# AcrylicShrimp/omok-ai

Hardware: AMD Instinct MI355X
Metric: self-play games/sec (15x15, 800 sims/move); MCTS nodes/sec (higher is better)
Workload: dtype f16x3 split MFMA, fp32 acc; fc0 corrections mixed f16/fp6; 1 GPU; 4096 concurrent 15x15 games per GPU, 800 sims/move, K=16, two trees per game; games_per_gpu=4096, board=15, sims_per_move=800, batch_k=16, warmup_step=whole episode, parallelism=games sharded x1, no hot-path collective

## Files before the change

### bindings/omok_mi355x.rs

```rust
#![allow(non_camel_case_types, dead_code)]

use std::ffi::{CStr, CString};
use std::os::raw::{c_char, c_int, c_void};
use std::ptr;

#[repr(C)]
#[derive(Clone, Copy, Debug)]
pub struct OmokConfig {
    pub board_size: i32,
    pub games: i32,
    pub max_nodes: i32,
    pub max_tables: i32,
    pub max_batch_k: i32,
    pub device: i32,
    pub net_mode: i32,
    pub max_tree_waves: i32,
    pub seed: u64,
    pub game_offset: i64,
}

#[repr(C)]
pub struct OmokEngine {
    _private: [u8; 0],
}
// ... 104 lines not shown
        pub fn omok_advance(e: *mut OmokEngine) -> c_int;
        pub fn omok_compute_policy(e: *mut OmokEngine, pi: *mut f32, has_policy: *mut u8) -> c_int;
        pub fn omok_play_actions(e: *mut OmokEngine, actions: *const i32) -> c_int;
        pub fn omok_set_actions(e: *mut OmokEngine, actions: *const i32) -> c_int;
        pub fn omok_selfplay_run(e: *mut OmokEngine, count: i32, batch_size: i32, epsilon: f32, alpha: f32, temperature: f32, threshold: i32, max_plies: i32, stats: *mut f64) -> c_int;
        pub fn omok_env_scripted_actions(e: *mut OmokEngine, kind: i32, boards: *const u8, turns: *const u8, batch: i32, forced_out: *mut i32) -> c_int;
        pub fn omok_opponent_actions(e: *mut OmokEngine, kind: i32, actions: *mut i32) -> c_int;
        pub fn omok_versus_run(e: *mut OmokEngine, kind: i32, opponent_side: i32, count: i32, batch_size: i32, epsilon: f32, alpha: f32, max_plies: i32, results: *mut i32, stats: *mut f64) -> c_int;
        pub fn omok_selfplay_run_slots(e: *mut OmokEngine, total_games: i32, count: i32, batch_size: i32, epsilon: f32, alpha: f32, temperature: f32, threshold: i32, records_dev: *mut c_void, cap_records: i64, game_offsets: *mut i64, game_lengths: *mut i32, game_status: *mut i32, n_records: *mut i64, stats: *mut f64) -> c_int;
        pub fn omok_round_generate(e: *mut OmokEngine, round: i32, batch_size: i32, epsilon: f32, alpha: f32, n_requests: *mut i32) -> c_int;
        pub fn omok_round_inputs(e: *mut OmokEngine, inputs: *mut f32) -> c_int;
        pub fn omok_round_eval(e: *mut OmokEngine) -> c_int;
        pub fn omok_round_outputs(e: *mut OmokEngine, p: *mut f32, v: *mut f32) -> c_int;
        pub fn omok_round_logits(e: *mut OmokEngine, logits: *mut f32, vpre: *mut f32) -> c_int;
        pub fn omok_round_inject(e: *mut OmokEngine, p: *const f32, v: *const f32) -> c_int;
        pub fn omok_round_scatter(e: *mut OmokEngine) -> c_int;
        pub fn omok_mirror_generate(e: *mut OmokEngine, n_requests: *mut i32) -> c_int;
        pub fn omok_mirror_inputs(e: *mut OmokEngine, inputs: *mut f32) -> c_int;
        pub fn omok_mirror_eval(e: *mut OmokEngine) -> c_int;
        pub fn omok_mirror_outputs(e: *mut OmokEngine, p: *mut f32) -> c_int;
        pub fn omok_mirror_inject(e: *mut OmokEngine, p: *const f32) -> c_int;
        pub fn omok_mirror_apply(e: *mut OmokEngine) -> c_int;
        pub fn omok_train_begin(e: *mut OmokEngine, max_batch: i32) -> c_int;
        pub fn omok_train_end(e: *mut OmokEngine) -> c_int;
        pub fn omok_train_step(e: *mut OmokEngine, records_dev: *const c_void, n_records: i64, indices: *const i64, batch: i32, losses: *mut f32) -> c_int;
        pub fn omok_train_losses(e: *mut OmokEngine, records_dev: *const c_void, n_records: i64, indices: *const i64, batch: i32, losses: *mut f32) -> c_int;
        pub fn omok_train_batch_indices(e: *mut OmokEngine, n_records: i64, batch: i32, key: u64, step: i32, out: *mut i64) -> c_int;
        pub fn omok_train_run(e: *mut OmokEngine, records_dev: *const c_void, n_records: i64, update_count: i32, batch_size: i32, key: u64, losses: *mut f32) -> c_int;
        pub fn omok_train_gradient_count(e: *const OmokEngine) -> i64;
        pub fn omok_train_backward(e: *mut OmokEngine, records_dev: *const c_void, n_records: i64, indices: *const i64, batch: i32, grad_dst_dev: *mut c_void) -> c_int;
        pub fn omok_train_apply(e: *mut OmokEngine, grads_dev: *const c_void, ranks: i32, losses: *mut f32) -> c_int;
        pub fn omok_debug_train_gradient(e: *mut OmokEngine, index: i32, out: *mut f32, count: i64) -> c_int;
        pub fn omok_net_read(e: *mut OmokEngine, index: i32, out: *mut f32, count: i64) -> c_int;
        pub fn omok_alive_count(e: *mut OmokEngine) -> c_int;
        pub fn omok_current_ply(e: *mut OmokEngine) -> c_int;
        pub fn omok_game_info(e: *mut OmokEngine, alive: *mut u8, status: *mut u8, plies: *mut i32) -> c_int;
        pub fn omok_tree_dump(e: *mut OmokEngine, game: i32, side: i32, ints: *mut i32, floats: *mut f32, cap_nodes: i32) -> c_int;
        pub fn omok_tree_root(e: *mut OmokEngine, game: i32, side: i32, root_n: *mut u32, root_w: *mut f32, n_nodes: *mut i32, n_tables: *mut i32) -> c_int;
        pub fn omok_root_stats(e: *mut OmokEngine, n: *mut u32, w: *mut f32) -> c_int;
        pub fn omok_root_children(e: *mut OmokEngine, game: i32, side: i32, actions: *mut i32, n: *mut u32, w: *mut f32, p: *mut f32, cap: i32) -> c_int;
        pub fn omok_replay_game(e: *mut OmokEngine, game: i32, boards: *mut u8, turns: *mut u8, pi: *mut f32, z: *mut f32, cap_plies: i32) -> c_int;
        pub fn omok_game_log_enable(e: *mut OmokEngine, enabled: i32) -> c_int;
        pub fn omok_game_log_read(e: *mut OmokEngine, first_game: i32, games: i32, start_boards: *mut u8, lengths: *mut i32, moves: *mut u16, root_n: *mut u32, root_w: *mut f32, child_n: *mut u32, child_w: *mut f32) -> c_int;
        pub fn omok_env_replay(e: *mut OmokEngine, start_boards: *const u8, moves: *const u16, lengths: *const i32, batch: i32, stride: i32, upto: i32, boards_out: *mut u8, status_out: *mut i32, played_out: *mut i32) -> c_int;
        pub fn omok_replay_pack_dev(e: *mut OmokEngine, dst_dev: *mut c_void, cap_records: i64) -> i64;
        pub fn omok_replay_record_bytes(e: *const OmokEngine) -> i32;
        pub fn omok_replay_augment_dev(e: *mut OmokEngine, dst_dev: *mut c_void, cap_records: i64) -> i64;
        pub fn omok_replay_augmented_game(e: *mut OmokEngine, game: i32, boards: *mut u8, turns: *mut u8, pi: *mut f32, z: *mut f32, cap_records: i32) -> c_int;
        pub fn omok_operand_row_bytes(e: *const OmokEngine) -> i64;
        pub fn omok_debug_operand_rows(e: *mut OmokEngine, first_row: i32, rows: i32, out: *mut c_void) -> c_int;
        pub fn omok_debug_set_base_cache(e: *mut OmokEngine, enabled: i32) -> c_int;
        pub fn omok_debug_set_children_kernel(e: *mut OmokEngine, which: i32) -> c_int;
        pub fn omok_debug_set_window_rects(e: *mut OmokEngine, enabled: i32) -> c_int;
        pub fn omok_debug_last_plan(e: *mut OmokEngine, out: *mut i32, cap: i32) -> c_int;
        pub fn omok_get_stats(e: *mut OmokEngine, stats: *mut f64) -> c_int;
        pub fn omok_reset_stats(e: *mut OmokEngine) -> c_int;
        pub fn omok_set_profiling(e: *mut OmokEngine, enabled: i32) -> c_int;
    }
}


#[repr(u8)]
#[derive(Clone, Copy, Debug, PartialEq, Eq)]
pub enum GameStatus {
    InProgress = 0,
    Draw = 1,
    BlackWin = 2,
    WhiteWin = 3,
}

impl GameStatus {
    pub fn from_raw(v: i32) -> Option<GameStatus> {
        match v {
            0 => Some(GameStatus::InProgress),
            1 => Some(GameStatus::Draw),
            2 => Some(GameStatus::BlackWin),
            3 => Some(GameStatus::WhiteWin),
            _ => None,
        }
    }
}

#[derive(Debug)]
pub struct OmokError {
    pub code: i32,
    pub message: String,
}

pub struct Engine {
    raw: *mut OmokEngine,
    hw: usize,
    games: usize,
}
unsafe impl Send for Engine {}

impl Engine {
    fn check(&self, rc: c_int) -> Result<c_int, OmokError> {
        if rc >= 0 {
            return Ok(rc);
        }
        let message = unsafe { CStr::from_ptr(ffi::omok_last_error(self.raw)) }.to_string_lossy().into_owned();
        Err(OmokError { code: rc, message })
    }

    pub fn new(cfg: &OmokConfig) -> Result<Engine, OmokError> {
        let mut raw: *mut OmokEngine = ptr::null_mut();
// ... 122 lines not shown
```

### include/omok_mi355x.h

```cpp
#ifndef OMOK_MI355X_H
#define OMOK_MI355X_H
#include <stdint.h>

#ifdef __cplusplus
extern "C" {
#endif

#define OMOK_OK 0
#define OMOK_ERR_INVALID (-1)
#define OMOK_ERR_HIP (-2)
#define OMOK_ERR_STATE (-3)
#define OMOK_ERR_OVERFLOW (-4)
#define OMOK_ERR_ILLEGAL (-5)

#define OMOK_MODE_PLAYER 0
#define OMOK_MODE_OPPONENT 1

#define OMOK_NET_F16X3 0
#define OMOK_NET_F32 1
#define OMOK_NET_F16X3_ROWS 2

#define OMOK_NET_F16X3_FP6 3
#define OMOK_NET_F16X3_F16 4
#define OMOK_NET_F16X3_MIXED 5
// ... 80 lines not shown
int omok_round_eval(omok_engine* e);
int omok_round_outputs(omok_engine* e, float* p, float* v);
int omok_round_logits(omok_engine* e, float* logits, float* vpre);
int omok_round_inject(omok_engine* e, const float* p, const float* v);
int omok_round_scatter(omok_engine* e);
int omok_mirror_generate(omok_engine* e, int32_t* n_requests);
int omok_mirror_inputs(omok_engine* e, float* inputs);
int omok_mirror_eval(omok_engine* e);
int omok_mirror_outputs(omok_engine* e, float* p);
int omok_mirror_inject(omok_engine* e, const float* p);
int omok_mirror_apply(omok_engine* e);

int omok_train_begin(omok_engine* e, int32_t max_batch);
int omok_train_end(omok_engine* e);
int omok_train_step(omok_engine* e, const void* records_dev, int64_t n_records, const int64_t* indices, int32_t batch, float* losses);
int omok_train_losses(omok_engine* e, const void* records_dev, int64_t n_records, const int64_t* indices, int32_t batch, float* losses);
int omok_train_batch_indices(omok_engine* e, int64_t n_records, int32_t batch, uint64_t key, int32_t step, int64_t* out);
int omok_train_run(omok_engine* e, const void* records_dev, int64_t n_records, int32_t update_count, int32_t batch_size, uint64_t key, float* losses);
#define OMOK_TRAIN_MAX_RANKS 64
int64_t omok_train_gradient_count(const omok_engine* e);
int omok_train_backward(omok_engine* e, const void* records_dev, int64_t n_records, const int64_t* indices, int32_t batch, void* grad_dst_dev);
int omok_train_apply(omok_engine* e, const void* grads_dev, int32_t ranks, float* losses);
int omok_debug_train_gradient(omok_engine* e, int32_t index, float* out, int64_t count);
int omok_net_read(omok_engine* e, int32_t index, float* out, int64_t count);

int omok_alive_count(omok_engine* e);
int omok_current_ply(omok_engine* e);
int omok_game_info(omok_engine* e, uint8_t* alive, uint8_t* status, int32_t* plies);
int omok_tree_dump(omok_engine* e, int32_t game, int32_t side, int32_t* ints, float* floats, int32_t cap_nodes);
int omok_tree_root(omok_engine* e, int32_t game, int32_t side, uint32_t* root_n, float* root_w,
                   int32_t* n_nodes, int32_t* n_tables);
int omok_root_stats(omok_engine* e, uint32_t* n, float* w);
int omok_root_children(omok_engine* e, int32_t game, int32_t side, int32_t* actions, uint32_t* n, float* w, float* p, int32_t cap);
int omok_replay_game(omok_engine* e, int32_t game, uint8_t* boards, uint8_t* turns, float* pi, float* z,
                     int32_t cap_plies);
#define OMOK_MOVE_CELL 255
#define OMOK_MOVE_EXTERNAL 256
int omok_game_log_enable(omok_engine* e, int32_t enabled);
int omok_game_log_read(omok_engine* e, int32_t first_game, int32_t games, uint8_t* start_boards, int32_t* lengths, uint16_t* moves,
                       uint32_t* root_n, float* root_w, uint32_t* child_n, float* child_w);
int omok_env_replay(omok_engine* e, const uint8_t* start_boards, const uint16_t* moves, const int32_t* lengths, int32_t batch,
                    int32_t stride, int32_t upto, uint8_t* boards_out, int32_t* status_out, int32_t* played_out);
int64_t omok_replay_pack_dev(omok_engine* e, void* dst_dev, int64_t cap_records);
int32_t omok_replay_record_bytes(const omok_engine* e);
int64_t omok_replay_augment_dev(omok_engine* e, void* dst_dev, int64_t cap_records);
int omok_replay_augmented_game(omok_engine* e, int32_t game, uint8_t* boards, uint8_t* turns, float* pi, float* z,
                               int32_t cap_records);

int64_t omok_operand_row_bytes(const omok_engine* e);
int omok_debug_operand_rows(omok_engine* e, int32_t first_row, int32_t rows, void* out);
int omok_debug_set_base_cache(omok_engine* e, int32_t enabled);
int omok_debug_set_children_kernel(omok_engine* e, int32_t which);
int omok_debug_set_window_rects(omok_engine* e, int32_t enabled);
#define OMOK_PLAN_INTS 16
int omok_debug_last_plan(omok_engine* e, int32_t* out, int32_t cap);

#define OMOK_STAT_SIMS 0
#define OMOK_STAT_EVALS 1
#define OMOK_STAT_PLY_GAMES 2
#define OMOK_STAT_FINISHED 3
#define OMOK_STAT_MS_TREE 4
#define OMOK_STAT_MS_TRUNK 5
#define OMOK_STAT_MS_FC0 6
#define OMOK_STAT_MS_TAIL 7
#define OMOK_STAT_MS_PLY 8
#define OMOK_STAT_FC0_LAUNCHES 9
#define OMOK_STAT_FC0_ROWS 10
#define OMOK_STAT_TREE_BYTES 11
#define OMOK_STAT_ROUND_LAUNCHES 12
#define OMOK_STAT_MS_ROUND 13
#define OMOK_STAT_PEAK_NODES 14
#define OMOK_STAT_PEAK_TABLES 15
#define OMOK_STAT_FC0_FORMAT 16
#define OMOK_STAT_PROBE_ROWS 17
#define OMOK_STAT_PROBE_DP_FP6 18
#define OMOK_STAT_PROBE_DV_FP6 19
#define OMOK_STAT_PROBE_DP_F16 20
#define OMOK_STAT_PROBE_DV_F16 21
#define OMOK_STAT_PROBE_LIMIT 22
#define OMOK_STAT_PROBE_LOGIT_MAX 23
#define OMOK_STAT_CHILDREN2_LAUNCHES 24
#define OMOK_STAT_CHILDREN1_LAUNCHES 25
#define OMOK_STAT_PROBE_DLOGIT_FP6 26
#define OMOK_STAT_PROBE_DLOGIT_F16 27
#define OMOK_STAT_PROBE_ROUND_ROWS 28
#define OMOK_STAT_PROBE_ROUND_FP6 29
#define OMOK_STAT_PROBE_ROUND_MIXED 32
#define OMOK_STAT_PROBE_ROUND_F16 35
#define OMOK_STAT_PROBE_LOGIT_LIMIT 38
#define OMOK_STAT_PROBE_OUTSIDE 39
#define OMOK_STAT_WORK_DIFF_RUNS 40
#define OMOK_STAT_WORK_DIFF_SINGLES 41
#define OMOK_STAT_WORK_DIFF_CHILDREN 42
#define OMOK_STAT_WORK_COPY_RUNS 43
#define OMOK_STAT_WORK_COPY_SINGLES 44
#define OMOK_STAT_WORK_COPY_CHILDREN 45
#define OMOK_STAT_WORK_DIFF_FULL_RUNS 46
#define OMOK_STAT_WORK_WIN_PIXELS 47
#define OMOK_STAT_WORK_WIN_TILES 48
#define OMOK_STAT_WORK_FULL_TILES 49
#define OMOK_STAT_MS_TRAIN_APPLY 50
#define OMOK_STAT_COUNT 51
int omok_get_stats(omok_engine* e, double* stats );
int omok_reset_stats(omok_engine* e);
int omok_set_profiling(omok_engine* e, int32_t enabled);

// ... 5 lines not shown
```

### omok-ai_amd/api.py

```python
import ctypes as C

import os

import numpy as np

from . import binding as B
from . import weights as W

EMPTY, BLACK, WHITE = 0, 1, 2
TURN_BLACK, TURN_WHITE = 0, 1
IN_PROGRESS, DRAW, BLACK_WIN, WHITE_WIN = 0, 1, 2, 3


class Engine:

    def __init__(self, board_size=15, games=1, max_nodes=2048, max_tables=1024, max_batch_k=16, device=0,
                 net_mode=B.NET_F16X3, seed=0, game_offset=0, max_tree_waves=0):
        self.n, self.hw, self.games = board_size, board_size * board_size, games
        self.max_nodes = max_nodes
        self.max_batch_k = max_batch_k
        cfg = B.Config(board_size, games, max_nodes, max_tables, max_batch_k, device, net_mode, max_tree_waves, seed, game_offset)
        h = C.c_void_p()
        rc = B.lib().omok_create(C.byref(cfg), C.byref(h))
        if rc != 0:
# ... 157 lines not shown
        forced = np.zeros(len(boards), dtype=np.int32)
        self._chk(B.lib().omok_env_scripted_actions(self.h, int(kind), B.u8ptr(boards), B.u8ptr(turns), len(boards), B.iptr(forced)))
        return forced

    def env_check_positions(self, boards):
        boards = np.ascontiguousarray(boards, dtype=np.uint8).reshape(-1, self.hw)
        verdict = np.zeros(len(boards), dtype=np.int32)
        stones = np.zeros(len(boards), dtype=np.int32)
        self._chk(B.lib().omok_env_check_positions(self.h, B.u8ptr(boards), len(boards), B.iptr(verdict), B.iptr(stones)))
        return verdict, stones

    def env_random_positions(self, key, first_game, stones, batch):
        boards = np.zeros((int(batch), self.hw), dtype=np.uint8)
        ok = np.zeros(int(batch), dtype=np.uint8)
        self._chk(B.lib().omok_env_random_positions(self.h, int(key) & 0xFFFFFFFFFFFFFFFF, int(first_game), int(stones), int(batch),
                                                    B.u8ptr(boards), B.u8ptr(ok)))
        return boards, ok

    def env_replay(self, start_boards, moves, lengths, upto=-1):
        moves = np.ascontiguousarray(moves, dtype=np.uint16)
        lengths = np.ascontiguousarray(lengths, dtype=np.int32).reshape(-1)
        batch = len(lengths)
        moves = moves.reshape(batch, -1)
        start = None
        if start_boards is not None:
            start = np.ascontiguousarray(start_boards, dtype=np.uint8).reshape(batch, self.hw)
        boards = np.zeros((batch, self.hw), dtype=np.uint8)
        status = np.zeros(batch, dtype=np.int32)
        played = np.zeros(batch, dtype=np.int32)
        self._chk(B.lib().omok_env_replay(self.h, None if start is None else B.u8ptr(start), moves.ctypes.data_as(C.POINTER(C.c_uint16)),
                                          B.iptr(lengths), batch, moves.shape[1], int(upto), B.u8ptr(boards), B.iptr(status), B.iptr(played)))
        return boards, status, played

    def encode_nn_input(self, boards, turns, mode=B.MODE_PLAYER):
        boards = np.ascontiguousarray(boards, dtype=np.uint8).reshape(-1, self.hw)
        turns = np.ascontiguousarray(turns, dtype=np.uint8).reshape(-1)
        out = np.zeros((boards.shape[0], 3 * self.hw), dtype=np.float32)
        self._chk(B.lib().omok_encode_nn_input(self.h, B.u8ptr(boards), B.u8ptr(turns), boards.shape[0], mode, B.fptr(out)))
        return out.reshape(-1, self.n, self.n, 3)

    def operand_rows(self, first_row, rows):
        nb = int(B.lib().omok_operand_row_bytes(self.h))
        if nb < 0:
            raise B.OmokError(nb, "no operand rows in this net mode")
        out = np.empty((rows, nb), dtype=np.uint8)
        self._chk(B.lib().omok_debug_operand_rows(self.h, first_row, rows, out.ctypes.data_as(C.c_void_p)))
        return out

    def set_base_cache(self, on=True):
        self._chk(B.lib().omok_debug_set_base_cache(self.h, int(bool(on))))

    def set_window_rects(self, on=True):
        self._chk(B.lib().omok_debug_set_window_rects(self.h, int(bool(on))))

    def set_children_kernel(self, which=2):
        self._chk(B.lib().omok_debug_set_children_kernel(self.h, int(which)))

    def last_plan(self):
        out = np.zeros(len(B.PLAN_NAMES), dtype=np.int32)
        n = self._chk(B.lib().omok_debug_last_plan(self.h, B.iptr(out), out.size))
        assert n == out.size
        d = dict(zip(B.PLAN_NAMES, (int(x) for x in out)))
        d["path"] = B.PLAN_PATHS[d["path"]]
        return d

    def set_profiling(self, on=True):
        self._chk(B.lib().omok_set_profiling(self.h, int(on)))

    def stats(self):
        s = (C.c_double * len(B.STAT_NAMES))()
        self._chk(B.lib().omok_get_stats(self.h, s))
        return dict(zip(B.STAT_NAMES, list(s)))

    def reset_stats(self):
        self._chk(B.lib().omok_reset_stats(self.h))


class Environment:

    def __init__(self, engine):
        self.eng = engine
        self._board = np.zeros((1, engine.hw), dtype=np.uint8)
        self._turn = np.zeros(1, dtype=np.uint8)
        self._legal = np.full(1, engine.hw, dtype=np.uint16)

    board = property(lambda s: s._board[0])
    turn = property(lambda s: int(s._turn[0]))
    legal_move_count = property(lambda s: int(s._legal[0]))

    def place_stone(self, index):
        s = int(self.eng.env_place_stone(self._board, self._turn, self._legal, [int(index)])[0])
        return None if s < 0 else s

    @staticmethod
    def check_positions(engine, boards):
        return engine.env_check_positions(boards)

    @staticmethod
    def random_positions(engine, key, first_game, stones, batch):
        return engine.env_random_positions(key, first_game, stones, batch)

    def encode_board(self, turn):
        t = np.array([turn], dtype=np.uint8)
        return self.eng.encode_nn_input(self.board[None], t, B.MODE_PLAYER).reshape(-1)[: 2 * self.eng.hw].copy()


# ... 271 lines not shown
```

### omok-ai_amd/binding.py

```python
import ctypes as C
import os
import subprocess

import numpy as np

_HERE = os.path.dirname(os.path.abspath(__file__))
LIB_PATH = os.environ.get("OMOK_MI355X_LIB") or os.path.join(_HERE, "libomok_mi355x.so")

OK = 0
NET_F16X3, NET_F32, NET_F16X3_ROWS, NET_F16X3_FP6, NET_F16X3_F16, NET_F16X3_MIXED = 0, 1, 2, 3, 4, 5
FC0_FORMATS = {-1: "f32", 0: "fp6", 1: "f16", 2: "mixed"}
MODE_PLAYER, MODE_OPPONENT = 0, 1
OPP_RANDOM, OPP_NAIVE = 0, 1
PLAN_NAMES = ["path", "rows", "nsplit", "tsplit", "runs", "singles", "run_rows", "full_runs", "tiles", "t_split", "ways", "fways",
              "fc0_format", "n_cu", "nsup", "reserved"]
PLAN_PATHS = {-1: "none", 0: "plain", 1: "copy", 2: "difference", 3: "f32"}
STAT_NAMES = ["sims", "evals", "ply_games", "finished", "ms_tree", "ms_trunk", "ms_fc0", "ms_tail", "ms_ply",
              "fc0_launches", "fc0_rows", "tree_bytes", "round_launches", "ms_round", "peak_nodes", "peak_tables",
              "fc0_format", "probe_rows", "probe_dp_fp6", "probe_dv_fp6", "probe_dp_f16", "probe_dv_f16", "probe_limit", "probe_logit_max",
              "children2_launches", "children1_launches", "probe_dlogit_fp6", "probe_dlogit_f16", "probe_round_rows",
              "probe_round_dp_fp6", "probe_round_dv_fp6", "probe_round_dlogit_fp6", "probe_round_dp_mixed", "probe_round_dv_mixed", "probe_round_dlogit_mixed",
              "probe_round_dp_f16", "probe_round_dv_f16", "probe_round_dlogit_f16", "probe_logit_limit", "probe_outside",
              "work_diff_runs", "work_diff_singles", "work_diff_children", "work_copy_runs", "work_copy_singles", "work_copy_children", "work_diff_full_runs",
              "work_win_pixels", "work_win_tiles", "work_full_tiles", "ms_train_apply"]

SYMBOLS = [
    "omok_create", "omok_destroy", "omok_last_error", "omok_net_num_tensors", "omok_net_tensor_size", "omok_net_load",
    "omok_net_commit", "omok_net_load_file", "omok_net_save_file", "omok_net2_load", "omok_net2_commit", "omok_net2_load_file", "omok_net2_info", "omok_match_reset", "omok_evaluate_pv", "omok_evaluate_logits", "omok_env_play", "omok_env_place_stone", "omok_encode_nn_input", "omok_selfplay_reset", "omok_set_episode", "omok_execute", "omok_execute_shared", "omok_execute_shared_recorded",
    "omok_compute_policy", "omok_play_actions", "omok_set_actions", "omok_root_children",
    "omok_env_scripted_actions", "omok_opponent_actions", "omok_versus_run",
    "omok_env_check_positions", "omok_selfplay_reset_from", "omok_root_stats",
    "omok_match_reset_from", "omok_env_random_positions",
    "omok_sample_actions", "omok_advance", "omok_selfplay_run", "omok_selfplay_run_slots", "omok_round_generate", "omok_round_inputs",
    "omok_round_eval", "omok_round_outputs", "omok_round_logits", "omok_round_inject", "omok_round_scatter", "omok_mirror_generate",
    "omok_mirror_inputs", "omok_mirror_eval", "omok_mirror_outputs", "omok_mirror_inject", "omok_mirror_apply",
    "omok_alive_count", "omok_current_ply", "omok_game_info", "omok_tree_dump", "omok_tree_root", "omok_replay_game",
    "omok_operand_row_bytes", "omok_debug_operand_rows", "omok_debug_set_base_cache", "omok_debug_set_children_kernel", "omok_debug_set_window_rects", "omok_debug_last_plan",
    "omok_replay_pack_dev", "omok_replay_record_bytes", "omok_replay_augment_dev", "omok_replay_augmented_game", "omok_get_stats", "omok_reset_stats", "omok_set_profiling",
    "omok_train_begin", "omok_train_end", "omok_train_step", "omok_train_losses", "omok_train_batch_indices", "omok_train_run",
    "omok_train_gradient_count", "omok_train_backward", "omok_train_apply",
    "omok_debug_train_gradient", "omok_net_read",
    "omok_game_log_enable", "omok_game_log_read", "omok_env_replay",
]


class Config(C.Structure):
    _fields_ = [("board_size", C.c_int32), ("games", C.c_int32), ("max_nodes", C.c_int32), ("max_tables", C.c_int32),
                ("max_batch_k", C.c_int32), ("device", C.c_int32), ("net_mode", C.c_int32), ("max_tree_waves", C.c_int32),
                ("seed", C.c_uint64), ("game_offset", C.c_int64)]


class OmokError(RuntimeError):
    def __init__(self, code, msg):
        super().__init__(f"omok error {code}: {msg}")
        self.code = code


def build():
    subprocess.check_call(["make", "-s", "-C", os.path.join(_HERE, "csrc")])


_lib = None


def lib():
    global _lib
    if _lib is not None:
        return _lib
    if not os.path.exists(LIB_PATH):
        raise OmokError(-2, f"{LIB_PATH} is missing: build it with __graft_entry__.build() (hipcc --offload-arch=gfx950); "
                            "there is no CPU fallback")
    L = C.CDLL(LIB_PATH)
    fp, ip = C.POINTER(C.c_float), C.POINTER(C.c_int32)
    u8p = C.POINTER(C.c_uint8)
    H = C.c_void_p
    L.omok_create.argtypes = [C.POINTER(Config), C.POINTER(H)]
    L.omok_destroy.argtypes = [H]
    L.omok_destroy.restype = None
    L.omok_last_error.argtypes = [H]
    L.omok_last_error.restype = C.c_char_p
    L.omok_net_tensor_size.argtypes = [H, C.c_int]
    L.omok_net_tensor_size.restype = C.c_int64
    L.omok_net_load.argtypes = [H, C.c_int, fp, C.c_int64]
    L.omok_net_commit.argtypes = [H]
    L.omok_net_load_file.argtypes = [H, C.c_char_p]
    L.omok_net_save_file.argtypes = [H, C.c_char_p]
    L.omok_net2_load.argtypes = [H, C.c_int, fp, C.c_int64]
    L.omok_net2_commit.argtypes = [H]
    L.omok_net2_load_file.argtypes = [H, C.c_char_p]
    L.omok_net2_info.argtypes = [H, ip, ip, C.POINTER(C.c_double)]
    L.omok_match_reset.argtypes = [H, C.c_int32]
    L.omok_evaluate_pv.argtypes = [H, fp, C.c_int32, fp, fp]
    L.omok_evaluate_logits.argtypes = [H, fp, C.c_int32, fp, fp]
    L.omok_env_play.argtypes = [H, ip, C.c_int32, C.c_int32, ip, u8p, u8p, C.POINTER(C.c_uint16)]
    L.omok_encode_nn_input.argtypes = [H, u8p, u8p, C.c_int32, C.c_int32, fp]
    L.omok_selfplay_reset.argtypes = [H]
    L.omok_execute_shared_recorded.argtypes = [H, C.c_int32, C.c_int32, C.c_float, C.c_float, C.c_int32, u8p, u8p, ip, fp, fp, C.c_int32, ip, ip]
    L.omok_operand_row_bytes.argtypes = [H]
    L.omok_operand_row_bytes.restype = C.c_int64
    L.omok_debug_operand_rows.argtypes = [H, C.c_int32, C.c_int32, C.c_void_p]
    L.omok_debug_set_base_cache.argtypes = [H, C.c_int32]
    L.omok_debug_set_children_kernel.argtypes = [H, C.c_int32]
    L.omok_debug_set_window_rects.argtypes = [H, C.c_int32]
    L.omok_debug_last_plan.argtypes = [H, ip, C.c_int32]
    L.omok_set_episode.argtypes = [H, C.c_uint64]
    L.omok_env_place_stone.argtypes = [H, u8p, u8p, C.POINTER(C.c_uint16), ip, C.c_int32, ip]
    L.omok_compute_policy.argtypes = [H, fp, u8p]
    L.omok_play_actions.argtypes = [H, ip]
    L.omok_set_actions.argtypes = [H, ip]
    L.omok_env_scripted_actions.argtypes = [H, C.c_int32, u8p, u8p, C.c_int32, ip]
    L.omok_opponent_actions.argtypes = [H, C.c_int32, ip]
    L.omok_versus_run.argtypes = [H, C.c_int32, C.c_int32, C.c_int32, C.c_int32, C.c_float, C.c_float, C.c_int32, ip, C.POINTER(C.c_double)]
    L.omok_env_check_positions.argtypes = [H, u8p, C.c_int32, ip, ip]
    L.omok_selfplay_reset_from.argtypes = [H, u8p]
    L.omok_match_reset_from.argtypes = [H, C.c_int32, u8p]
    L.omok_env_random_positions.argtypes = [H, C.c_uint64, C.c_int64, C.c_int32, C.c_int32, u8p, u8p]
    L.omok_root_stats.argtypes = [H, C.POINTER(C.c_uint32), fp]
    L.omok_root_children.argtypes = [H, C.c_int32, C.c_int32, ip, C.POINTER(C.c_uint32), fp, fp, C.c_int32]
    L.omok_execute.argtypes = [H, C.c_int32, C.c_int32, C.c_float, C.c_float]
    L.omok_execute_shared.argtypes = [H, C.c_int32, C.c_int32, C.c_float, C.c_float, C.c_int32]
    L.omok_sample_actions.argtypes = [H, C.c_float, C.c_int32, ip]
    L.omok_advance.argtypes = [H]
    L.omok_selfplay_run.argtypes = [H, C.c_int32, C.c_int32, C.c_float, C.c_float, C.c_float, C.c_int32, C.c_int32,
                                    C.POINTER(C.c_double)]
    L.omok_selfplay_run_slots.argtypes = [H, C.c_int32, C.c_int32, C.c_int32, C.c_float, C.c_float, C.c_float, C.c_int32, C.c_void_p, C.c_int64,
                                          C.POINTER(C.c_int64), ip, ip, C.POINTER(C.c_int64), C.POINTER(C.c_double)]
    L.omok_round_generate.argtypes = [H, C.c_int32, C.c_int32, C.c_float, C.c_float, ip]
    L.omok_round_inputs.argtypes = [H, fp]
    L.omok_round_eval.argtypes = [H]
    L.omok_round_outputs.argtypes = [H, fp, fp]
    L.omok_round_logits.argtypes = [H, fp, fp]
    L.omok_round_inject.argtypes = [H, fp, fp]
    L.omok_round_scatter.argtypes = [H]
    L.omok_mirror_generate.argtypes = [H, ip]
    L.omok_mirror_inputs.argtypes = [H, fp]
    L.omok_mirror_eval.argtypes = [H]
    L.omok_mirror_outputs.argtypes = [H, fp]
    L.omok_mirror_inject.argtypes = [H, fp]
    L.omok_mirror_apply.argtypes = [H]
    L.omok_alive_count.argtypes = [H]
    L.omok_current_ply.argtypes = [H]
    L.omok_game_info.argtypes = [H, u8p, u8p, ip]
    L.omok_tree_dump.argtypes = [H, C.c_int32, C.c_int32, ip, fp, C.c_int32]
    L.omok_tree_root.argtypes = [H, C.c_int32, C.c_int32, C.POINTER(C.c_uint32), fp, ip, ip]
    L.omok_replay_game.argtypes = [H, C.c_int32, u8p, u8p, fp, fp, C.c_int32]
    L.omok_replay_pack_dev.argtypes = [H, C.c_void_p, C.c_int64]
    L.omok_replay_pack_dev.restype = C.c_int64
    L.omok_replay_augment_dev.argtypes = [H, C.c_void_p, C.c_int64]
    L.omok_replay_augment_dev.restype = C.c_int64
    L.omok_replay_augmented_game.argtypes = [H, C.c_int32, u8p, u8p, fp, fp, C.c_int32]
    L.omok_replay_record_bytes.argtypes = [H]
    L.omok_get_stats.argtypes = [H, C.POINTER(C.c_double)]
    L.omok_reset_stats.argtypes = [H]
    L.omok_set_profiling.argtypes = [H, C.c_int32]
    i64p = C.POINTER(C.c_int64)
    L.omok_train_begin.argtypes = [H, C.c_int32]
# ... 30 lines not shown
```

### omok-ai_amd/csrc/common.h

```cpp
#pragma once
#include <hip/hip_runtime.h>
#include <stdint.h>

namespace omok {

constexpr uint16_t NONE16 = 0xFFFFu;
constexpr uint8_t NONE8 = 0xFFu;
constexpr int KMAX = 64;
constexpr float F32_EPS = 1.1920928955078125e-7f;

enum { ST_IN_PROGRESS = 0, ST_DRAW = 1, ST_BLACK_WIN = 2, ST_WHITE_WIN = 3 };
enum { RNG_EXPAND = 1, RNG_NOISE = 2, RNG_SAMPLE = 3, RNG_OPPONENT = 4, RNG_TRAIN_BATCH = 5 };

template <int N>
struct Geo {
    static constexpr int HW = N * N;
    static constexpr int ROWP = (HW + 63) / 64 * 64;
    static constexpr int NW = (HW + 63) / 64;
    static constexpr int IT = ROWP / 64;
};

struct __attribute__((aligned(16))) NodeHdr {
    uint16_t parent;
    uint16_t table;
// ... 48 lines not shown
    uint32_t* req_aux;
    int32_t* d_count;
    uint64_t* rp_board;
    uint8_t* rp_turn;
    float* rp_pi;
    float* rp_z;
    unsigned long long* d_bytes;
    int cap_nodes, cap_tables, games;
    int stride_nodes, stride_tables;
};

struct RoundArgs {
    int side, round, K, ply;
    float epsilon, alpha;
    uint64_t seed;
    int64_t game_offset;
    const float* scatter_v;
};

void launch_reset(int n, const Store& S, const float* root_policy_dev , hipStream_t st);
void launch_reset_from(int n, const Store& S, const uint8_t* boards_dev, const float* p_dev, const float* p2_dev, int split, hipStream_t st);
void launch_random_positions(int n, uint64_t key, int64_t first_game, int stones, int batch, uint8_t* boards_dev, uint8_t* ok_dev, hipStream_t st);
void launch_position_check(int n, const uint8_t* boards_dev, int batch, int32_t* verdict_dev, int32_t* stones_dev, hipStream_t st);
struct GameLog {
    uint32_t* root_n;
    float* root_w;
    uint32_t* child_n;
    float* child_w;
    uint16_t* move;
    uint8_t* start_board;
};
void launch_log_move(int n, const Store& S, int side, int start_ply, const GameLog& L, hipStream_t st);
void launch_replay(int n, const uint8_t* start_dev, const int32_t* verdict_dev, const uint16_t* moves_dev, const int32_t* lengths_dev, int batch, int stride,
                   int upto, uint8_t* boards_out, int32_t* status_out, int32_t* played_out, hipStream_t st);
void launch_root_stats(const Store& S, int side, uint32_t* n_dev, float* w_dev, hipStream_t st);
struct SlotMeta { long long offset; int32_t len; int32_t status; };
void launch_harvest(int n, const Store& S, uint8_t* mask_dev , long long* slot_off_dev , long long* out_count_dev, SlotMeta* meta_dev,
                    uint8_t* dst_dev, long long cap_records, hipStream_t st);
void launch_refill(int n, const Store& S, const float* root_policy_dev, int32_t* next_gid_dev, int total_games, int32_t* new_gid_dev , hipStream_t st);
void launch_round(int n, const Store& S, const RoundArgs& a, hipStream_t st);
void launch_fill(const Store& S, int side, int K, hipStream_t st);
void launch_scan(int n, const Store& S, int side, int K, hipStream_t st, unsigned long long* evals_dev = nullptr, int32_t* zero_ptr = nullptr, int zero_n = 0,
                 bool fill = true);
void launch_round_shared(int n, const Store& S, const RoundArgs& a, int rounds_total, int group, int waves, uint16_t* sh_req, uint32_t* sh_cnt,
                         hipStream_t st, uint8_t* rec_order = nullptr, uint32_t* rec_pos = nullptr);
void launch_scatter_shared(int n, const Store& S, int side, const float* p_dev, const float* v_dev, int max_count, int waves, const uint16_t* sh_req,
                           const uint32_t* sh_cnt, hipStream_t st, uint8_t* rec_order = nullptr, uint32_t* rec_pos = nullptr);
constexpr int MAX_TREE_WAVES = 16;
constexpr int MAX_GAMES = 32767;
constexpr int SCAN_GAMES_PER_THREAD = 32;
void launch_scatter(int n, const Store& S, int side, const float* p_dev, const float* v_dev, int max_count, hipStream_t st, bool backups = true);
void launch_backups(int n, const Store& S, int side, const float* v_dev, hipStream_t st);
void launch_softmax_scatter(int n, const Store& S, int side, const float* logits_dev, int lrow, float* v_dev, float* vpre_dev, int max_count,
                            hipStream_t st, bool backups = true);
void launch_sample(int n, const Store& S, int side, int ply, float temperature, int threshold, uint64_t seed,
                   int64_t game_offset, int32_t* actions_dev, hipStream_t st);
void launch_mirror_scan(int n, const Store& S, int side, hipStream_t st);
void launch_advance(int n, const Store& S, int side, const float* p_dev, hipStream_t st);
void launch_encode_requests(int n, const Store& S, float* out_dev , int max_b, hipStream_t st);
void launch_env_play(int n, const int32_t* moves_dev, int batch, int len, int32_t* status_dev, uint8_t* boards_dev,
                     uint8_t* turns_dev, uint16_t* legal_dev, hipStream_t st);
void launch_encode_boards(int n, const uint8_t* boards_dev, const uint8_t* turns_dev, int batch, int mode,
                          float* out_dev, hipStream_t st);
void launch_replay_pack(int n, const Store& S, const long long* offsets_dev, uint8_t* dst_dev, long long cap_records, hipStream_t st);
void launch_replay_offsets(int n, const Store& S, int per_transition, long long* offsets_dev , hipStream_t st);
void launch_set_actions(int n, const Store& S, int side, const int32_t* actions_dev, uint32_t* d_flags , hipStream_t st);
void launch_clear_actions(const Store& S, hipStream_t st);
void launch_opponent_move(int n, const Store& S, int side, int kind, uint64_t seed, int64_t game_offset, int32_t* actions_dev, hipStream_t st);
void launch_env_scripted(int n, const uint8_t* boards_dev, int kind, int batch, int32_t* forced_dev, hipStream_t st);
void launch_policy(int n, const Store& S, int side, float* pi_dev , uint8_t* has_dev , hipStream_t st);
void launch_env_place(int n, uint8_t* boards_dev, uint8_t* turns_dev, uint16_t* legal_dev, const int32_t* actions_dev, int batch,
                      int32_t* status_dev, hipStream_t st);
int set_advance_lds_attribute(int n, size_t bytes);
void launch_replay_augment(int n, const Store& S, const long long* offsets_dev, int game_first, int game_count, long long base_sub,
                           uint8_t* dst_dev, long long cap_records, hipStream_t st);
size_t advance_lds_bytes(int cap_nodes, int cap_tables);

void launch_match_split(const Store& S, int tree_side, int split, uint32_t* ref2, uint32_t* aux2, int32_t* cnt, unsigned long long* evals, int max_rows,
                        hipStream_t st);
void launch_match_join(const int32_t* cnt, const float* v2, float* v1, const float* p2, float* p1, int rowp, int max_rows, hipStream_t st);
void launch_match_roots(int n, const Store& S, const float* root_policy2, int split, hipStream_t st);

struct NetBuffers;
}
```

### omok-ai_amd/csrc/engine.cpp

```cpp
#include "../../include/omok_mi355x.h"
#include "common.h"
#include "net.h"
#include "train.h"

#include <algorithm>
#include <cstdarg>
#include <cstdio>
#include <cstring>
#include <string>
#include <vector>

using namespace omok;

hipEvent_t Prof::get() {
    if (n_pool > 0) return pool[--n_pool];
    hipEvent_t e;
    hipEventCreate(&e);
    return e;
}
void Prof::begin(int cat, hipStream_t st) {
    if (!enabled || !active) return;
    if (n_items == cap_items) {
        if (cap_items >= 8192) resolve();
        else {
// ... 263 lines not shown
    rc |= dalloc(e, &e->d_sh_cnt, 2 * (size_t)KMAX);
    rc |= dalloc(e, &e->d_flags, 4);
    rc |= dalloc(e, &e->d_pi, G * HW);
    rc |= dalloc(e, &e->d_has, G);
    rc |= dalloc(e, &e->d_aug_offsets, G + 1);
    if (rc) {
        g_create_error = e->err;
        omok_destroy(e);
        return OMOK_ERR_HIP;
    }
    hipMemsetAsync(S.d_count, 0, 16, e->st);
    hipMemsetAsync(S.d_bytes, 0, 16, e->st);
    hipMemsetAsync(e->d_error, 0, 16, e->st);
    hipMemsetAsync(e->d_evals, 0, 16, e->st);
    hipMemsetAsync(S.gs, 0, sizeof(GameState) * G, e->st);
    hipMemsetAsync(S.ts, 0, sizeof(TreeState) * T, e->st);
    if (set_advance_lds_attribute(e->n, advance_lds_bytes(cfg->max_nodes, cfg->max_tables)) != 0) {
        g_create_error = "hipFuncSetAttribute(k_advance, max dynamic LDS) failed";
        omok_destroy(e);
        return OMOK_ERR_HIP;
    }
    configure_net(e, e->net, (int)max_b);
    if (net_alloc(e->net) == 0) {
        g_create_error = "net buffer allocation failed (hipMalloc)";
        omok_destroy(e);
        return OMOK_ERR_HIP;
    }
    if (hipStreamSynchronize(e->st) != hipSuccess) {
        g_create_error = "stream sync failed after init";
        omok_destroy(e);
        return OMOK_ERR_HIP;
    }
    *out = e;
    return OMOK_OK;
}

extern "C" int omok_net_num_tensors(void) { return NET_TENSORS; }
extern "C" int64_t omok_net_tensor_size(const omok_engine* e, int index) { return e ? net_tensor_size(e->n, index) : -1; }

static int sync_and_check(omok_engine* e, const char* what);

static int net2_alloc(omok_engine* e) {
    if (e->net2) return 0;
    const size_t mb = (size_t)e->net.max_b;
    if (!e->d_mref && dalloc(e, &e->d_mref, mb)) return OMOK_ERR_HIP;
    if (!e->d_maux && dalloc(e, &e->d_maux, mb)) return OMOK_ERR_HIP;
    if (!e->d_mcnt && dalloc(e, &e->d_mcnt, 4)) return OMOK_ERR_HIP;
    if (!e->d_mevals && dalloc(e, &e->d_mevals, 2)) return OMOK_ERR_HIP;
    if (!e->d_root_policy2 && dalloc(e, &e->d_root_policy2, (size_t)e->rowp)) return OMOK_ERR_HIP;
    HIPCHK(e, hipMemset(e->d_mcnt, 0, 16));
    HIPCHK(e, hipMemset(e->d_mevals, 0, 16));
    Net* n2 = new Net();
    configure_net(e, *n2, e->net.max_b);
    if (net_alloc(*n2) == 0) { delete n2; return fail(e, OMOK_ERR_HIP, "net 2 buffer allocation failed (hipMalloc)"); }
    e->net2 = n2;
    return 0;
}

static int net_load_slot(omok_engine* e, int slot, int index, const float* data, int64_t count) {
    if (!e || !data) return OMOK_ERR_INVALID;
    if (index < 0 || index >= NET_TENSORS) return fail(e, OMOK_ERR_INVALID, "tensor index %d out of range", index);
    if (count != e->net.wsize[index]) return fail(e, OMOK_ERR_INVALID, "tensor %d: expected %lld values, got %lld", index, (long long)e->net.wsize[index], (long long)count);
    HIPCHK(e, hipSetDevice(e->cfg.device));
    if (slot == 2 && net2_alloc(e)) return OMOK_ERR_HIP;
    Net& net = slot == 2 ? *e->net2 : e->net;
    HIPCHK(e, hipMemcpyAsync(net.w[index], data, sizeof(float) * (size_t)count, hipMemcpyHostToDevice, e->st));
    HIPCHK(e, hipStreamSynchronize(e->st));
    net.loaded[index] = true;
    net.committed = false;
    return OMOK_OK;
}

static int net_commit_slot(omok_engine* e, int slot) {
    if (!e) return OMOK_ERR_INVALID;
    if (slot == 2 && !e->net2) return fail(e, OMOK_ERR_STATE, "net 2: no tensor was ever loaded");
    Net& net = slot == 2 ? *e->net2 : e->net;
    for (int i = 0; i < NET_TENSORS; ++i)
        if (!net.loaded[i]) return fail(e, OMOK_ERR_STATE, "tensor %d was never loaded", i);
    HIPCHK(e, hipSetDevice(e->cfg.device));
    if (e->round_reqs >= 0 || e->mirror_reqs >= 0) return fail(e, OMOK_ERR_STATE, "omok_net_commit while a round / mirror batch is pending");
    if (net_commit(net, e->S, e->st) != 0) return fail(e, OMOK_ERR_HIP, "weight packing / format probe failed");
    net_invalidate_sibling_cache(net);
    HIPCHK(e, hipStreamSynchronize(e->st));
    net.committed = true;
    return OMOK_OK;
}

extern "C" int omok_net_load(omok_engine* e, int index, const float* data, int64_t count) { return net_load_slot(e, 1, index, data, count); }
extern "C" int omok_net_commit(omok_engine* e) { return net_commit_slot(e, 1); }
extern "C" int omok_net2_load(omok_engine* e, int index, const float* data, int64_t count) { return net_load_slot(e, 2, index, data, count); }
extern "C" int omok_net2_commit(omok_engine* e) { return net_commit_slot(e, 2); }

extern "C" int omok_net2_info(omok_engine* e, int32_t* fc0_format, int32_t* probe_outside, double* evals) {
    if (!e) return OMOK_ERR_INVALID;
    if (!e->net2 || !e->net2->committed) return fail(e, OMOK_ERR_STATE, "net 2 not loaded/committed (omok_net2_load x31 + omok_net2_commit)");
    ENTER(e);
    const Net& n2 = *e->net2;
    if (fc0_format) *fc0_format = n2.mode == OMOK_NET_F32 ? -1 : (n2.diff_fp6 ? FC0_MIXED : n2.fc0_fmt);
    if (probe_outside) *probe_outside = n2.probe_outside;
    if (evals) {
        unsigned long long ev[2] = {0, 0};
        if (sync_and_check(e, "net2_info")) return OMOK_ERR_HIP;
        HIPCHK(e, hipMemcpy(ev, e->d_mevals, sizeof(ev), hipMemcpyDeviceToHost));
        evals[0] = (double)ev[0];
        evals[1] = (double)ev[1];
    }
// ... 54 lines not shown
    }
    fclose(f);
    for (int i = 0; rc == OMOK_OK && i < NET_TENSORS; ++i) rc = net_load_slot(e, slot, i, params[i].data(), (int64_t)params[i].size());
    if (rc != OMOK_OK) return rc;
    return net_commit_slot(e, slot);
}
extern "C" int omok_net_load_file(omok_engine* e, const char* path) { return net_load_file_slot(e, 1, path); }
extern "C" int omok_net2_load_file(omok_engine* e, const char* path) { return net_load_file_slot(e, 2, path); }

extern "C" int omok_net_save_file(omok_engine* e, const char* path) {
    if (!e || !path) return OMOK_ERR_INVALID;
    for (int i = 0; i < NET_TENSORS; ++i)
        if (!e->net.loaded[i]) return fail(e, OMOK_ERR_STATE, "tensor %d was never loaded", i);
    HIPCHK(e, hipSetDevice(e->cfg.device));
    FILE* f = fopen(path, "wb");
    if (!f) return fail(e, OMOK_ERR_INVALID, "cannot create weights file %s", path);
    bool ok = wr_u64(f, NET_TENSORS);
    char name[64];
    for (int i = 0; ok && i < NET_TENSORS; ++i) {
        net_tensor_name(i, name, sizeof(name));
        const size_t len = strlen(name);
        ok = wr_u64(f, len) && fwrite(name, 1, len, f) == len;
    }
    ok = ok && wr_u64(f, NET_TENSORS);
    std::vector<float> buf;
    for (int i = 0; ok && i < NET_TENSORS; ++i) {
        const size_t len = (size_t)e->net.wsize[i];
        buf.resize(len);
        if (hipMemcpy(buf.data(), e->net.w[i], sizeof(float) * len, hipMemcpyDeviceToHost) != hipSuccess) { fclose(f); return fail(e, OMOK_ERR_HIP, "weight read-back failed"); }
        ok = wr_u64(f, len) && fwrite(buf.data(), sizeof(float), len, f) == len;
    }
    ok = (fclose(f) == 0) && ok;
    return ok ? OMOK_OK : fail(e, OMOK_ERR_INVALID, "short write to %s", path);
}

static int need_net(omok_engine* e) {
    if (!e->net.committed) return fail(e, OMOK_ERR_STATE, "net not loaded/committed (omok_net_load x31 + omok_net_commit)");
    if (e->match && !e->net2->committed) return fail(e, OMOK_ERR_STATE, "match episode: net 2 was reloaded and not committed (omok_net2_commit)");
    return 0;
}

static Net& net_at(omok_engine* e, int idx) { return idx == 0 ? e->net : *e->net2; }
static void invalidate_nets(omok_engine* e) {
    net_invalidate_sibling_cache(e->net);
    if (e->net2) net_invalidate_sibling_cache(*e->net2);
}
static bool block_live(const omok_engine* e, int b) { return b == 0 ? e->split > 0 : e->split < e->cfg.games; }
static Store block_view(const omok_engine* e, int b) {
    Store V = e->S;
    if (b == 0) V.d_count = e->d_mcnt;
    else { V.req_ref = e->d_mref; V.req_aux = e->d_maux; V.d_count = e->d_mcnt + 1; }
    return V;
}
static void match_forward(omok_engine* e, int b, int tree_side, int max_count, int sibling_side, bool skip_softmax) {
    Net& X = net_at(e, tree_side ^ b);
    X.grp_lo = b ? e->split : 0;
    X.grp_hi = b ? e->cfg.games : e->split;
    X.grp_sub = b ? e->d_mcnt : nullptr;
    net_forward_requests(X, block_view(e, b), max_count, e->st, &e->prof, sibling_side, skip_softmax);
    X.grp_hi = -1;
    X.grp_sub = nullptr;
}
static void match_split(omok_engine* e, int tree_side, int max_rows) {
    launch_match_split(e->S, tree_side, e->split, e->d_mref, e->d_maux, e->d_mcnt, e->d_mevals, max_rows, e->st);
}
static void match_join(omok_engine* e, int tree_side, bool p, int max_rows) {
    if (!block_live(e, 1)) return;
    Net &A = net_at(e, tree_side), &B = net_at(e, tree_side ^ 1);
    launch_match_join(e->d_mcnt, B.v, A.v, p ? B.p : nullptr, p ? A.p : nullptr, e->rowp, max_rows, e->st);
}
static int match_counts(omok_engine* e) {
    HIPCHK(e, hipMemcpyAsync(e->match_cnt, e->d_mcnt, sizeof(e->match_cnt), hipMemcpyDeviceToHost, e->st));
    return sync_and_check(e, "match counts") ? OMOK_ERR_HIP : 0;
}
static int no_match(omok_engine* e, const char* what) {
    if (e->match) return fail(e, OMOK_ERR_STATE, "%s is not available in a match episode (omok_match_reset): start self-play with omok_selfplay_reset", what);
    return 0;
}

static int check_async(omok_engine* e, const char* what) {
    hipError_t r = hipGetLastError();
    if (r != hipSuccess) return fail(e, OMOK_ERR_HIP, "%s: launch failed: %s", what, hipGetErrorString(r));
    return 0;
}

static int sync_and_check(omok_engine* e, const char* what) {
    hipError_t r = hipStreamSynchronize(e->st);
    if (r != hipSuccess) return fail(e, OMOK_ERR_HIP, "%s: %s", what, hipGetErrorString(r));
    return check_async(e, what);
}

extern "C" int omok_net_read(omok_engine* e, int32_t index, float* out, int64_t count) {
    if (!e || !out) return OMOK_ERR_INVALID;
    if (index < 0 || index >= NET_TENSORS) return fail(e, OMOK_ERR_INVALID, "tensor index %d out of range", index);
    if (count != e->net.wsize[index]) return fail(e, OMOK_ERR_INVALID, "tensor %d: expected %lld values, got %lld", index, (long long)e->net.wsize[index], (long long)count);
    if (!e->net.loaded[index]) return fail(e, OMOK_ERR_STATE, "tensor %d was never loaded", index);
    ENTER(e);
    if (sync_and_check(e, "net_read")) return OMOK_ERR_HIP;
    HIPCHK(e, hipMemcpy(out, e->net.w[index], sizeof(float) * (size_t)count, hipMemcpyDeviceToHost));
    return OMOK_OK;
}

extern "C" int omok_train_end(omok_engine* e) {
    ENTER(e);
    if (!e->train) return OMOK_OK;
    if (sync_and_check(e, "train_end")) return OMOK_ERR_HIP;
    train_free(*e->train);
    delete e->train;
    e->train = nullptr;
    return OMOK_OK;
}

extern "C" int omok_train_begin(omok_engine* e, int32_t max_batch) {
    if (!e) return OMOK_ERR_INVALID;
// ... 387 lines not shown
}

extern "C" int omok_selfplay_reset_from(omok_engine* e, const uint8_t* boards) {
    if (!e || !boards) return OMOK_ERR_INVALID;
    if (!e->net.committed) return fail(e, OMOK_ERR_STATE, "net not loaded/committed (omok_net_load x31 + omok_net_commit)");
    ENTER(e);
    return reset_from_positions(e, boards, false, 0);
}

extern "C" int omok_match_reset_from(omok_engine* e, int32_t split, const uint8_t* boards) {
    if (!e || !boards) return OMOK_ERR_INVALID;
    if (!e->net.committed) return fail(e, OMOK_ERR_STATE, "net not loaded/committed (omok_net_load x31 + omok_net_commit)");
    if (!e->net2 || !e->net2->committed) return fail(e, OMOK_ERR_STATE, "net 2 not loaded/committed (omok_net2_load x31 + omok_net2_commit)");
    if (split < 0 || split > e->cfg.games) return fail(e, OMOK_ERR_INVALID, "split %d outside [0, games = %d]", split, e->cfg.games);
    ENTER(e);
    return reset_from_positions(e, boards, true, split);
}

extern "C" int omok_env_random_positions(omok_engine* e, uint64_t key, int64_t first_game, int32_t stones, int32_t batch, uint8_t* boards_out,
                                         uint8_t* ok_out) {
    if (!e || !boards_out || !ok_out) return OMOK_ERR_INVALID;
    if (stones < 0 || stones >= e->hw) return fail(e, OMOK_ERR_INVALID, "stones %d outside [0, %d)", stones, e->hw);
    if (batch < 1) return fail(e, OMOK_ERR_INVALID, "batch %d < 1", batch);
    ENTER(e);
    uint8_t* d_out = nullptr;
    const size_t B = (size_t)batch;
    HIPCHK(e, hipMalloc((void**)&d_out, B * e->hw + B));
    e->prof.begin(PC_PLY, e->st);
    launch_random_positions(e->n, key, first_game, stones, batch, d_out, d_out + B * e->hw, e->st);
    e->prof.end(e->st);
    hipMemcpyAsync(boards_out, d_out, B * e->hw, hipMemcpyDeviceToHost, e->st);
    hipMemcpyAsync(ok_out, d_out + B * e->hw, B, hipMemcpyDeviceToHost, e->st);
    const int rc = sync_and_check(e, "env_random_positions");
    hipFree(d_out);
    return rc ? OMOK_ERR_HIP : OMOK_OK;
}

static int need_reset(omok_engine* e) {
    if (!e->reset_done) return fail(e, OMOK_ERR_STATE, "omok_selfplay_reset has not been called");
    return 0;
}

static void enqueue_match_round(omok_engine* e, int side, int K, bool eval_and_scatter, int alive, bool defer_backups) {
    const int max_req = std::min(alive * K, e->net.max_b);
    launch_scan(e->n, e->S, side, K, e->st, e->d_evals);
    match_split(e, side, max_req);
    e->prof.end(e->st);
    if (!eval_and_scatter) return;
    for (int b = 0; b < 2; ++b) {
        if (!block_live(e, b)) continue;
        Net& X = net_at(e, side ^ b);
        const Store V = block_view(e, b);
        const bool fused = net_logits_cover_batch(X, alive * K);
        match_forward(e, b, side, alive * K, side, fused);
        e->prof.begin(PC_TREE_OTHER, e->st);
        if (fused) {
            int lrow = 0;
            const float* lg = net_logits(X, &lrow);
            launch_softmax_scatter(e->n, V, side, lg, lrow, X.v, X.vpre, alive * K, e->st, false);
        } else launch_scatter(e->n, V, side, X.p, X.v, alive * K, e->st, false);
        e->prof.end(e->st);
    }
    e->prof.begin(PC_TREE_OTHER, e->st);
    match_join(e, side, false, max_req);
    if (!defer_backups) launch_backups(e->n, e->S, side, net_at(e, side).v, e->st);
    e->prof.end(e->st);
}

static Net& backup_net(omok_engine* e, int side) { return e->match ? net_at(e, side) : e->net; }

static void enqueue_round(omok_engine* e, int round, int K, float eps, float alpha, bool eval_and_scatter, int alive, bool defer_backups = false,
                          bool pending_backups = false) {
    const int side = e->ply & 1;
    RoundArgs a{side, round, K, e->ply, eps, alpha, e->key, e->cfg.game_offset, pending_backups ? backup_net(e, side).v : nullptr};
    e->prof.round_begin();
    e->prof.begin(PC_ROUND, e->st);
    launch_round(e->n, e->S, a, e->st);
    e->prof.end(e->st);
    e->prof.begin(PC_TREE_OTHER, e->st);
    if (e->match) {
        enqueue_match_round(e, side, K, eval_and_scatter, alive, defer_backups);
        e->prof.round_end();
        return;
    }
    int max_req = alive * K;
    if (max_req > e->net.max_b) max_req = e->net.max_b;
    const bool sib_round = eval_and_scatter && net_round_takes_sibling_path(e->net, max_req);
    launch_scan(e->n, e->S, side, K, e->st, e->d_evals, sib_round ? e->net.d_gcnt : nullptr, NET_GCNT_INTS, !sib_round);
    e->net.gcnt_zeroed = e->net.fill_in_group = sib_round;
    e->net.fill_side = side;
    e->net.fill_k = K;
    e->prof.end(e->st);
    if (eval_and_scatter) {
        const bool fused = net_logits_cover_batch(e->net, alive * K);
        net_forward_requests(e->net, e->S, alive * K, e->st, &e->prof, side, fused);
        e->prof.begin(PC_TREE_OTHER, e->st);
        if (fused) {
            int lrow = 0;
            const float* lg = net_logits(e->net, &lrow);
            launch_softmax_scatter(e->n, e->S, side, lg, lrow, e->net.v, e->net.vpre, alive * K, e->st, !defer_backups);
        } else launch_scatter(e->n, e->S, side, e->net.p, e->net.v, alive * K, e->st, !defer_backups);
        e->prof.end(e->st);
    }
    e->prof.round_end();
}

static int enqueue_execute(omok_engine* e, int count, int K, float eps, float alpha, int alive) {
    int processed = 0, round = 0;
    while (processed < count) {
        enqueue_round(e, round, K, eps, alpha, true, alive, true, round > 0);
        processed += K;
        round += 1;
    }
    if (round > 0) {
        e->prof.begin(PC_TREE_OTHER, e->st);
        launch_backups(e->n, e->S, e->ply & 1, backup_net(e, e->ply & 1).v, e->st);
        e->prof.end(e->st);
    }
    return round;
}

static int check_exec_args(omok_engine* e, int count, int K, float eps, float alpha) {
    if (count < 1) return fail(e, OMOK_ERR_INVALID, "count must be >= 1");
    if (K < 1 || K > e->cfg.max_batch_k) return fail(e, OMOK_ERR_INVALID, "batch_size %d outside [1, max_batch_k=%d]", K, e->cfg.max_batch_k);
    if (!(alpha > 0.0f)) return fail(e, OMOK_ERR_INVALID, "alpha must be > 0");
    if (!(eps >= 0.0f && eps <= 1.0f)) return fail(e, OMOK_ERR_INVALID, "epsilon must be in [0,1]");
    return 0;
}

extern "C" int omok_execute(omok_engine* e, int32_t count, int32_t batch_size, float epsilon, float alpha) {
    if (!e) return OMOK_ERR_INVALID;
    if (need_net(e) || need_reset(e)) return OMOK_ERR_STATE;
    if (check_exec_args(e, count, batch_size, epsilon, alpha)) return OMOK_ERR_INVALID;
    HIPCHK(e, hipSetDevice(e->cfg.device));
    uint32_t bits = 0, alive = 0;
    if (read_status(e, &bits, &alive)) return OMOK_ERR_HIP;
    const int rounds = enqueue_execute(e, count, batch_size, epsilon, alpha, (int)alive);
    e->sims += (double)rounds * batch_size * alive;
    if (read_status(e, &bits, &alive)) return OMOK_ERR_HIP;
    return tree_error(e, bits);
}

extern "C" int omok_execute_shared(omok_engine* e, int32_t count, int32_t batch_size, float epsilon, float alpha, int32_t waves) {
    if (!e) return OMOK_ERR_INVALID;
    if (need_net(e) || need_reset(e)) return OMOK_ERR_STATE;
    if (check_exec_args(e, count, batch_size, epsilon, alpha)) return OMOK_ERR_INVALID;
    if (no_match(e, "omok_execute_shared")) return OMOK_ERR_STATE;
    if (e->cfg.games != 1) return fail(e, OMOK_ERR_INVALID, "omok_execute_shared searches ONE tree: create the engine with games = 1 (got %d)", e->cfg.games);
    if (waves < 1 || waves > MAX_TREE_WAVES || waves * batch_size > e->net.max_b)
        return fail(e, OMOK_ERR_INVALID, "waves must be in [1, %d] and waves * batch_size <= %d (the net batch, sized by max(games, max_tree_waves = %d) * max_batch_k)",
                    MAX_TREE_WAVES, e->net.max_b, e->cfg.max_tree_waves);
    HIPCHK(e, hipSetDevice(e->cfg.device));
    uint32_t bits = 0, alive = 0;
// ... 908 lines not shown
    launch_replay_offsets(e->n, e->S, 6, e->d_aug_offsets, e->st);
    launch_replay_augment(e->n, e->S, e->d_aug_offsets, 0, e->cfg.games, 0, (uint8_t*)dst_dev, cap_records, e->st);
    long long total = 0;
    if (hipMemcpyAsync(&total, e->d_aug_offsets + e->cfg.games, 8, hipMemcpyDeviceToHost, e->st) != hipSuccess) return OMOK_ERR_HIP;
    if (sync_and_check(e, "replay_augment")) return OMOK_ERR_HIP;
    return total;
}

extern "C" int omok_replay_augmented_game(omok_engine* e, int32_t game, uint8_t* boards, uint8_t* turns, float* pi, float* z, int32_t cap_records) {
    if (!e || game < 0 || game >= e->cfg.games || cap_records < 0) return OMOK_ERR_INVALID;
    HIPCHK(e, hipSetDevice(e->cfg.device));
    const size_t hw = (size_t)e->hw, brd = (hw + 1 + 3) / 4 * 4, rec = brd + 4 * hw + 4, max_rec = 6 * hw;
    if (!e->d_aug_scratch && dalloc(e, &e->d_aug_scratch, max_rec * rec)) return OMOK_ERR_HIP;
    long long off[2] = {0, 0};
    launch_replay_offsets(e->n, e->S, 6, e->d_aug_offsets, e->st);
    HIPCHK(e, hipMemcpyAsync(off, e->d_aug_offsets + game, 16, hipMemcpyDeviceToHost, e->st));
    if (sync_and_check(e, "replay_augmented_game")) return OMOK_ERR_HIP;
    const int total = (int)(off[1] - off[0]);
    const int n = total < cap_records ? total : cap_records;
    if (n <= 0) return total;
    launch_replay_augment(e->n, e->S, e->d_aug_offsets, game, 1, off[0], e->d_aug_scratch, (long long)max_rec, e->st);
    std::vector<uint8_t> host((size_t)total * rec);
    HIPCHK(e, hipMemcpyAsync(host.data(), e->d_aug_scratch, host.size(), hipMemcpyDeviceToHost, e->st));
    if (sync_and_check(e, "replay_augmented_game")) return OMOK_ERR_HIP;
    for (int i = 0; i < n; ++i) {
        const uint8_t* r = host.data() + (size_t)i * rec;
        if (boards) memcpy(boards + (size_t)i * hw, r, hw);
        if (turns) turns[i] = r[hw];
        if (pi) memcpy(pi + (size_t)i * hw, r + brd, 4 * hw);
        if (z) memcpy(z + i, r + brd + 4 * hw, 4);
    }
    return total;
}

extern "C" int64_t omok_operand_row_bytes(const omok_engine* e) { return e && e->net.mode != OMOK_NET_F32 ? (int64_t)e->net.row_u4 * 16 : OMOK_ERR_INVALID; }
extern "C" int omok_debug_operand_rows(omok_engine* e, int32_t first_row, int32_t rows, void* out) {
    if (!e || !out || first_row < 0 || rows < 0 || first_row + rows > e->net.max_b || e->net.mode == OMOK_NET_F32) return OMOK_ERR_INVALID;
    ENTER(e);
    HIPCHK(e, hipMemcpyAsync(out, (const char*)e->net.a_fc0 + (size_t)first_row * e->net.row_u4 * 16, (size_t)rows * e->net.row_u4 * 16, hipMemcpyDeviceToHost, e->st));
    return sync_and_check(e, "debug_operand_rows") ? OMOK_ERR_HIP : OMOK_OK;
}

extern "C" int omok_debug_set_base_cache(omok_engine* e, int32_t enabled) {
    if (!e) return OMOK_ERR_INVALID;
    e->net.base_cache = enabled != 0;
    net_invalidate_sibling_cache(e->net);
    return OMOK_OK;
}

extern "C" int omok_debug_set_window_rects(omok_engine* e, int32_t enabled) {
    if (!e) return OMOK_ERR_INVALID;
    e->net.win_rects = enabled != 0;
    return OMOK_OK;
}

extern "C" int omok_debug_set_children_kernel(omok_engine* e, int32_t which) {
    if (!e) return OMOK_ERR_INVALID;
    if (which != 1 && which != 2) return fail(e, OMOK_ERR_INVALID, "children kernel %d (1 = k_sib_children, 2 = k_sib_children2)", which);
    if (which == 1 && e->net.mode != OMOK_NET_F32 && e->net.diff_fp6)
        return fail(e, OMOK_ERR_STATE, "omok_debug_set_children_kernel(1): the engine runs the mixed operand format, whose difference path exists in k_sib_children2 only "
                                       "(create the engine with OMOK_NET_F16X3_FP6 or _F16 to compare the two kernels)");
    e->net.sib_v2 = which == 2;
    net_invalidate_sibling_cache(e->net);
    return OMOK_OK;
}

extern "C" int omok_debug_last_plan(omok_engine* e, int32_t* out, int32_t cap) {
    if (!e || !out || cap < 0) return OMOK_ERR_INVALID;
    ENTER(e);
    const Net& net = e->net;
    int32_t plan[OMOK_PLAN_INTS] = {};
    plan[0] = net.plan_path; plan[1] = net.plan_rows; plan[2] = net.plan_nsplit; plan[3] = net.plan_tsplit;
    plan[12] = net.mode == OMOK_NET_F32 ? -1 : net.diff_fp6 ? FC0_MIXED : net.fc0_fmt;
    plan[13] = net.n_cu;
    plan[14] = 2 * net.hw;
    if (sync_and_check(e, "debug_last_plan")) return OMOK_ERR_HIP;
    if ((net.plan_path == 1 || net.plan_path == 2) && net.d_gcnt) {
        int32_t c[NET_GCNT_HEAD_INTS];
        HIPCHK(e, hipMemcpy(c, net.d_gcnt, sizeof(c), hipMemcpyDeviceToHost));
        plan[4] = c[NET_GCNT_RUNS]; plan[5] = c[NET_GCNT_SINGLES]; plan[6] = c[NET_GCNT_ROWS_IN_RUNS];
        if (net.plan_path == 2) {
            plan[7] = c[NET_GCNT_FULL_EVALS]; plan[8] = c[NET_GCNT_WIN_TILES]; plan[9] = c[NET_GCNT_SPLIT_TILE0]; plan[10] = c[NET_GCNT_WIN_WAYS];
            plan[11] = c[NET_GCNT_FULL_WAYS];
        }
    }
    const int n = cap < OMOK_PLAN_INTS ? cap : OMOK_PLAN_INTS;
    for (int i = 0; i < n; ++i) out[i] = plan[i];
    return n;
}

extern "C" int omok_get_stats(omok_engine* e, double* stats) {
    if (!e || !stats) return OMOK_ERR_INVALID;
    HIPCHK(e, hipSetDevice(e->cfg.device));
    if (sync_and_check(e, "get_stats")) return OMOK_ERR_HIP;
    e->prof.resolve();
    unsigned long long ev = 0, by = 0;
    HIPCHK(e, hipMemcpy(&ev, e->d_evals, 8, hipMemcpyDeviceToHost));
    HIPCHK(e, hipMemcpy(&by, e->S.d_bytes, 8, hipMemcpyDeviceToHost));
    for (int i = 0; i < OMOK_STAT_COUNT; ++i) stats[i] = 0.0;
    stats[OMOK_STAT_SIMS] = e->sims;
    stats[OMOK_STAT_EVALS] = e->evals + (double)ev;
    stats[OMOK_STAT_PLY_GAMES] = e->ply_games;
    stats[OMOK_STAT_FINISHED] = e->finished;
    stats[OMOK_STAT_MS_TREE] = e->prof.total_ms(PC_ROUND) + e->prof.total_ms(PC_TREE_OTHER);
    stats[OMOK_STAT_MS_TRUNK] = e->prof.total_ms(PC_TRUNK);
    stats[OMOK_STAT_MS_FC0] = e->prof.total_ms(PC_FC0);
// ... 59 lines not shown
```

### omok-ai_amd/csrc/net.h

```cpp
#pragma once
#include "common.h"
#include "../../include/omok_mi355x.h"

namespace omok {

constexpr int NET_TENSORS = 31;
constexpr int NC = 128;
constexpr int NM = 32;
constexpr int NF = 512;
enum { FC0_AUTO = -1, FC0_FP6 = 0, FC0_F16 = 1, FC0_MIXED = 2 };
constexpr float NET_PROBE_LIMIT = 3e-4f;
constexpr float NET_PROBE_LOGIT_LIMIT = 5e-4f;
constexpr float NET_PROBE_CONTRACT = 1e-3f;
constexpr int NET_PROBE_ROWS = 2048;

struct Net {
    int n = 0, hw = 0, rowp = 0, mode = 0;
    int cfg_mode = 0;
    bool siblings = true;
    int device = 0;
    int max_b = 0;
    bool committed = false;
    bool loaded[NET_TENSORS] = {};
    int64_t wsize[NET_TENSORS] = {};
    float* w[NET_TENSORS] = {};
    float* p = nullptr;
    float* v = nullptr;
    float* vpre = nullptr;
    float* in_f32 = nullptr;
    int chunk = 0;
    float *sx = nullptr, *sh = nullptr, *sd = nullptr, *sg = nullptr, *s0 = nullptr, *s1 = nullptr;
    float *s0_x3 = nullptr, *s0_f32 = nullptr;
    int probe_outside = 0;
    void* wt_trunk = nullptr;
    float* wt_first = nullptr;
    void* wt_fc0 = nullptr;
    void* wt_fc1 = nullptr;
    void* wt_heads = nullptr;
    void* a_fc0 = nullptr;
    void* h0 = nullptr;
    size_t row_u4 = 0;
    size_t part_rows = 0;
    float* part = nullptr;
    void* d_groups = nullptr;
    int32_t* d_singles = nullptr;
    void* d_sib_rows = nullptr;
    int32_t* d_gcnt = nullptr;
    unsigned long long* d_work = nullptr;
    float* sib_h = nullptr;
    uint32_t* d_sib_slot = nullptr;
    int32_t* d_bin_start = nullptr;
    int32_t* d_tile_info = nullptr;
    void* d_slot_desc = nullptr;
    void* d_rows = nullptr;
    size_t d_slots = 0;
    int games = 0;
    size_t base_slots = 0;
    void* a_base = nullptr;
    float* facc = nullptr;
    int32_t* d_tags = nullptr;
    void* d_comp = nullptr;
    bool gcnt_zeroed = false;
    bool fill_in_group = false;
    int fill_side = 0, fill_k = 0;
    double children_launches[2] = {0.0, 0.0};
    bool sib_v2 = true;
    bool win_rects = true;
    bool base_cache = true;
    bool sib_cache_valid = false;
    float* part_w = nullptr;
    size_t part_w_rows = 0;
    int n_cu = 256;
    int mx_sw = 0;
    int fc0_policy = FC0_AUTO;
    int fc0_fmt = 0;
    bool diff_fp6 = false;
    void* wt_fc0x = nullptr;
    size_t row_u4_fmt[2] = {0, 0};
    float probe[24] = {};
    size_t bytes = 0;
    int grp_lo = 0, grp_hi = -1;
    const int32_t* grp_sub = nullptr;
    int plan_path = -1, plan_rows = 0, plan_nsplit = 0, plan_tsplit = 0;
};

inline int64_t net_tensor_size(int n, int idx) {
    const int64_t hw = (int64_t)n * n;
    if (idx == 0) return 3 * NC;
    if (idx == 1) return NC;
    if (idx >= 2 && idx < 23) {
        const int64_t q[7] = {NC * NM, NM, 9 * NM, NM * NM, NM, NM * NC, NC};
        return q[(idx - 2) % 7];
    }
    switch (idx) {
        case 23: return NC * hw * NF;
        case 24: return NF;
        case 25: return (int64_t)NF * NF;
        case 26: return NF;
        case 27: return NF;
        case 28: return 1;
        case 29: return NF * hw;
        case 30: return hw;
    }
    return -1;
}

bool net_logits_cover_batch(const Net& net, int max_count);
bool net_round_takes_sibling_path(const Net& net, int max_count);
enum {
    NET_GCNT_RUNS = 0,
    NET_GCNT_SINGLES = 1,
    NET_GCNT_ROWS_IN_RUNS = 2,
    NET_GCNT_FULL_ROWS = 3,
    NET_GCNT_WIN_TILES = 4,
    NET_GCNT_SPLIT_TILE0 = 5,
    NET_GCNT_WIN_WAYS = 6,
    NET_GCNT_TILE_ORDER = 7,
    NET_GCNT_BINS = 8,
    NET_GCNT_FULL_EVALS = 96,
    NET_GCNT_UNCACHEABLE = 97,
    NET_GCNT_FULL_WAYS = 98,
    NET_GCNT_FULL_STRIDE = 99,
    NET_GCNT_HEAD_INTS = 100
};
constexpr int NET_GCNT_P0 = 8 + 81 + 7 + 16;
constexpr int NET_GCNT_INTS = NET_GCNT_P0 + 225;
constexpr int NET_WORK_DIFF = 0, NET_WORK_COPY = 3, NET_WORK_DIFF_FULL = 6, NET_WORK_WIN_PIXELS = 7, NET_WORK_WIN_TILES = 8, NET_WORK_FULL_TILES = 9, NET_WORK_COUNT = 16;
void net_forward_requests(Net& net, const Store& S, int max_count, hipStream_t st, struct Prof* prof, int sibling_side = -1, bool skip_softmax = false);
void net_forward_inputs(Net& net, const Store& S, int count, hipStream_t st, struct Prof* prof);
inline void net_invalidate_sibling_cache(Net& net) { net.sib_cache_valid = false; }
int net_commit(Net& net, const Store& S, hipStream_t st);
void net_set_fc0_format(Net& net, int fmt);
const float* net_logits(const Net& net, int* row_stride);
size_t net_alloc(Net& net);
void net_free(Net& net);

enum { PC_ROUND = 0, PC_TREE_OTHER, PC_TRUNK, PC_FC0, PC_TAIL, PC_PLY, PC_TRAIN_APPLY, PC_COUNT };
constexpr int PC_COUNT_MAX = 8;
struct Prof {
    bool enabled = false;
    int every = 1;
    long long rounds_seen = 0, rounds_timed = 0;
    bool active = true;
    bool in_round = false;
    double ms_s[PC_COUNT_MAX] = {};
    long long launches_s[PC_COUNT_MAX] = {};
    void round_begin() { in_round = true; active = every <= 1 || rounds_seen % every == 0; ++rounds_seen; if (active) ++rounds_timed; }
    void round_end() { in_round = false; active = true; }
    double scale() const { return rounds_timed > 0 ? (double)rounds_seen / (double)rounds_timed : 1.0; }
    double total_ms(int cat) const { return ms[cat] + ms_s[cat] * scale(); }
    double total_launches(int cat) const { return (double)launches[cat] + (double)launches_s[cat] * scale(); }
    struct Item { int cat; bool sampled; hipEvent_t a, b; };
    Item* items = nullptr;
    int n_items = 0, cap_items = 0;
    hipEvent_t* pool = nullptr;
    int n_pool = 0, cap_pool = 0;
    double ms[PC_COUNT] = {};
    long long launches[PC_COUNT] = {};
    hipEvent_t get();
    void begin(int cat, hipStream_t st);
    void end(hipStream_t st);
    void resolve();
    void destroy();
};

}
```

### omok-ai_amd/csrc/net_kernels.hip

```cpp
#include "net.h"

#include <cmath>
#include <cstdlib>
#include <cstring>
#include <vector>

namespace omok {

typedef _Float16 half8 __attribute__((ext_vector_type(8)));
typedef float f32x16 __attribute__((ext_vector_type(16)));
typedef float f32x4 __attribute__((ext_vector_type(4)));

enum { EPI_SPLIT = 0, EPI_LOGITS = 1, EPI_PARTIAL = 2 };
constexpr int GT_BS = 128;

__host__ __device__ inline int kperm(int T, int s, int h, int j) { return 32 * T + 16 * s + 8 * (j >> 2) + 4 * h + (j & 3); }
__device__ inline float lrelu(float x) {
    const float y = 0.2f * x;
    float r;
    asm("v_max_f32 %0, %1, %2" : "=v"(r) : "v"(x), "v"(y));
    return r;
}

typedef _Float16 half2v __attribute__((ext_vector_type(2)));
typedef unsigned int u32x4 __attribute__((ext_vector_type(4)));
__device__ inline void nt_store(const uint4& v, uint4* p) { __builtin_nontemporal_store(u32x4{v.x, v.y, v.z, v.w}, (u32x4*)p); }
__device__ inline uint4 nt_load(const uint4* p) { const u32x4 v = __builtin_nontemporal_load((const u32x4*)p); return make_uint4(v[0], v[1], v[2], v[3]); }
typedef unsigned int u32x6 __attribute__((ext_vector_type(6)));
typedef float f32x16v __attribute__((ext_vector_type(16)));
typedef _Float16 half32 __attribute__((ext_vector_type(32)));
typedef float f32x2 __attribute__((ext_vector_type(2)));
__device__ inline void split8(const float* v, half8& hi, half8& lo) {
    union { uint32_t u[4]; half8 h; } H, L;
#pragma unroll
    for (int j = 0; j < 4; ++j) {
        const float a = v[2 * j], b = v[2 * j + 1];
        const uint32_t ph = __builtin_bit_cast(uint32_t, __builtin_convertvector((f32x2){a, b}, half2v));
        uint32_t pl;
        asm("v_fma_mixlo_f16 %0, %1, -1.0, %2 op_sel_hi:[1,0,0]" : "=v"(pl) : "v"(ph), "v"(a));
        asm("v_fma_mixhi_f16 %0, %1, -1.0, %2 op_sel:[1,0,0] op_sel_hi:[1,0,0]" : "+v"(pl) : "v"(ph), "v"(b));
        H.u[j] = ph;
        L.u[j] = pl;
    }
    hi = H.h;
    lo = L.h;
}
__device__ inline f32x2 lrelu2(float a, float b) {
    const f32x2 y = (f32x2){a, b} * 0.2f;
    f32x2 r;
    asm("v_max_f32 %0, %1, %2" : "=v"(r[0]) : "v"(a), "v"(y[0]));
    asm("v_max_f32 %0, %1, %2" : "=v"(r[1]) : "v"(b), "v"(y[1]));
    return r;
}
// ... 2490 lines not shown
    const int wm = wave >> 1, ws = wave & 1;
    const int h = lane >> 5;
    const int kbeg = EPI == EPI_PARTIAL ? (int)blockIdx.y * ksteps : 0;
    f32x16 acc[MTW][2];
    gemm_t_mainloop<MT, NST, 0>(lds, wp, act, ksteps, kbeg, act_row_u4, k_full, last_cnt, lo_off, b0, wave, lane, acc, [](int) {});

#pragma unroll
    for (int c = 0; c < 2; ++c) {
        const int sample = b0 + 32 * (2 * ws + c) + (lane & 31);
        if (sample >= count) continue;
#pragma unroll
        for (int i = 0; i < MTW; ++i) {
            const int mt = wm * MTW + i;
            float y[16];
#pragma unroll
            for (int g = 0; g < 4; ++g) {
                const f32x4 bv = *(const f32x4*)(bias + 32 * mt + 8 * g + 4 * h);
#pragma unroll
                for (int q = 0; q < 4; ++q) y[4 * g + q] = acc[i][c][4 * g + q] + bv[q];
            }
            if (EPI == EPI_PARTIAL) {
#pragma unroll
                for (int g = 0; g < 4; ++g) {
                    f32x4 o;
#pragma unroll
                    for (int q = 0; q < 4; ++q) o[q] = acc[i][c][4 * g + q];
                    *(f32x4*)(out_logits + ((size_t)blockIdx.y * out_row_u4 + sample) * (MT * 32) + 32 * mt + 8 * g + 4 * h) = o;
                }
            } else if (EPI == EPI_SPLIT) {
#pragma unroll
                for (int s = 0; s < 2; ++s) {
                    float v[8];
#pragma unroll
                    for (int j = 0; j < 8; ++j) v[j] = lrelu(y[8 * s + j]);
                    half8 hi, lo;
                    split8(v, hi, lo);
                    uint4* row = out_split + (size_t)sample * out_row_u4 + (size_t)(2 * mt + s) * 4;
                    row[h] = *(const uint4*)&hi;
                    row[2 + h] = *(const uint4*)&lo;
                }
            } else {
#pragma unroll
                for (int g = 0; g < 4; ++g) {
                    f32x4 o;
#pragma unroll
                    for (int q = 0; q < 4; ++q) o[q] = y[4 * g + q];
                    *(f32x4*)(out_logits + (size_t)sample * (MT * 32) + 32 * mt + 8 * g + 4 * h) = o;
                }
            }
        }
    }
}

template <int MTH>
__global__ __launch_bounds__(512) void k_tail_fused(const uint4* __restrict__ wp_fc1, const uint4* __restrict__ act, const float* __restrict__ bias_fc1,
                                                    const uint4* __restrict__ wp_heads, const float* __restrict__ bias_heads, float* __restrict__ out_logits,
                                                    const int32_t* __restrict__ d_count, int max_count) {
    constexpr int MTW = MTH / 4;
    constexpr int WFR = MTH * 2;
    constexpr int LPW = WFR / 8;
    constexpr int FC1_STAGE_U4 = 40 * 64;
    constexpr int H0_U4 = 2 * FC1_STAGE_U4, HST_U4 = WFR * 64;
    constexpr int CHUNK_U4 = 96 * 64;
    static_assert(WFR % 8 == 0 && 2 * HST_U4 <= FC1_STAGE_U4 && H0_U4 + HST_U4 <= CHUNK_U4, "heads ring inside the freed fc1 slots");
    extern __shared__ __attribute__((aligned(16))) unsigned char smem[];
    uint4* lds = (uint4*)smem;
    int count = d_count[0];
    if (count > max_count) count = max_count;
    const int b0 = blockIdx.x * GT_BS;
    if (b0 >= count) return;
    const int tid = threadIdx.x, lane = tid & 63;
    const int wave = __builtin_amdgcn_readfirstlane(tid >> 6);
    const int wm = wave >> 1, ws = wave & 1;
    const int h = lane >> 5;

    const uint4* hsrc = wp_heads + (size_t)wave * 64 + lane;
    auto hslot = [&](int slot) { return lds + (slot == 0 ? H0_U4 : (slot - 1) * HST_U4); };
    auto hissue_one = [&](int ks, int slot, int i) { dma16(hsrc + (size_t)ks * (WFR * 64) + i * 8 * 64, hslot(slot) + (wave + 8 * i) * 64); };
    auto hissue = [&](int ks, int slot) {
#pragma unroll
        for (int i = 0; i < LPW; ++i) hissue_one(ks, slot, i);
    };

    uint4 fr[4][2][2][2];
    {
        f32x16 acc[4][2];
        gemm_t_mainloop<16, 3, LPW>(lds, wp_fc1, act, 32, 0, 128, 32, 1, 2, b0, wave, lane, acc, [&](int j) { hissue(j, j); });
#pragma unroll
        for (int i = 0; i < 4; ++i) {
            const int mt = wm * 4 + i;
            f32x4 bv[4];
#pragma unroll
            for (int g = 0; g < 4; ++g) bv[g] = *(const f32x4*)(bias_fc1 + 32 * mt + 8 * g + 4 * h);
#pragma unroll
            for (int c = 0; c < 2; ++c) {
                float y[16];
#pragma unroll
                for (int g = 0; g < 4; ++g)
#pragma unroll
                    for (int q = 0; q < 4; ++q) y[4 * g + q] = acc[i][c][4 * g + q] + bv[g][q];
#pragma unroll
                for (int s = 0; s < 2; ++s) {
                    float v[8];
#pragma unroll
                    for (int j = 0; j < 8; ++j) v[j] = lrelu(y[8 * s + j]);
                    half8 hi, lo;
                    split8(v, hi, lo);
                    fr[i][c][s][0] = *(const uint4*)&hi;
                    fr[i][c][s][1] = *(const uint4*)&lo;
                }
            }
            __builtin_amdgcn_sched_barrier(0);
        }
    }

    f32x16 acc[MTW][2];
#pragma unroll
    for (int i = 0; i < MTW; ++i)
#pragma unroll
        for (int c = 0; c < 2; ++c)
#pragma unroll
            for (int r = 0; r < 16; ++r) acc[i][c][r] = 0.0f;
    uint4* chunk = lds + CHUNK_U4;
    int slot = 0, nslot = 2;
    for (int p = 0; p < 4; ++p) {
        if (p) {
            asm volatile("s_waitcnt lgkmcnt(0)" ::: "memory");
            __builtin_amdgcn_s_barrier();
            asm volatile("" ::: "memory");
        }
        if (wm == p) {
#pragma unroll
            for (int i = 0; i < 4; ++i)
#pragma unroll
                for (int s = 0; s < 2; ++s)
#pragma unroll
                    for (int c = 0; c < 2; ++c)
#pragma unroll
                        for (int part = 0; part < 2; ++part) chunk[(((2 * i + s) * 4 + 2 * ws + c) * 2 + part) * 64 + lane] = fr[i][c][s][part];
        }
        asm volatile("s_waitcnt lgkmcnt(0)" ::: "memory");
        for (int kk = 0; kk < 8; ++kk) {
            const int ks = 8 * p + kk;
            if (ks < 31) asm volatile("s_waitcnt vmcnt(%0) lgkmcnt(0)" ::"n"(LPW) : "memory");
            else asm volatile("s_waitcnt vmcnt(0) lgkmcnt(0)" ::: "memory");
            __builtin_amdgcn_s_barrier();
            asm volatile("" ::: "memory");
            const bool stage = ks + 2 < 32;
            const half8* L = (const half8*)hslot(slot);
            const half8* C = (const half8*)chunk + (size_t)(kk * 8) * 64 + lane;
            half8 bh[2], bl[2], ah[MTW], al[MTW];
#pragma unroll
            for (int c = 0; c < 2; ++c) {
                bh[c] = C[((2 * ws + c) * 2 + 0) * 64];
                bl[c] = C[((2 * ws + c) * 2 + 1) * 64];
            }
#pragma unroll
            for (int i = 0; i < MTW; ++i) {
                ah[i] = L[((wm * MTW + i) * 2 + 0) * 64 + lane];
                al[i] = L[((wm * MTW + i) * 2 + 1) * 64 + lane];
            }
#pragma unroll
            for (int term = 0; term < 3; ++term)
#pragma unroll
                for (int i = 0; i < MTW; ++i) {
#pragma unroll
                    for (int c = 0; c < 2; ++c) acc[i][c] = MFMA16(term == 1 ? al[i] : ah[i], term == 2 ? bl[c] : bh[c], acc[i][c]);
                    if (stage && term == 0) {
#pragma unroll
                        for (int q = i; q < LPW; q += MTW) hissue_one(ks + 2, nslot, q);
                    }
                }
            slot = slot + 1 == 3 ? 0 : slot + 1;
            nslot = nslot + 1 == 3 ? 0 : nslot + 1;
        }
    }

#pragma unroll
    for (int c = 0; c < 2; ++c) {
        const int sample = b0 + 32 * (2 * ws + c) + (lane & 31);
        if (sample >= count) continue;
#pragma unroll
        for (int i = 0; i < MTW; ++i) {
            const int mt = wm * MTW + i;
#pragma unroll
            for (int g = 0; g < 4; ++g) {
                const f32x4 bv = *(const f32x4*)(bias_heads + 32 * mt + 8 * g + 4 * h);
                f32x4 o;
#pragma unroll
                for (int q = 0; q < 4; ++q) o[q] = acc[i][c][4 * g + q] + bv[q];
                *(f32x4*)(out_logits + (size_t)sample * (MTH * 32) + 32 * mt + 8 * g + 4 * h) = o;
            }
        }
    }
}

constexpr int GW_DA = 3, GW_NB = 3;
constexpr int gemm_w_lds(int mt) { return (8 * GW_DA * (mt / 8) * 2 + GW_NB * 16) * 1024; }
template <int MT, int EPI>
__global__ __launch_bounds__(512) void k_gemm_w(const uint4* __restrict__ wp, const uint4* __restrict__ act, int ksteps, size_t act_row_u4,
                                                const float* __restrict__ bias, uint4* __restrict__ out_split, size_t out_row_u4,
                                                float* __restrict__ out_logits, const int32_t* __restrict__ d_count, int max_count) {
    static_assert(MT % 8 == 0 && EPI != EPI_PARTIAL, "k_gemm_w: whole-K launches of at least one m-tile per wave");
    constexpr int MTW = MT / 8;
    constexpr int AF = MTW * 2;
    constexpr int B_U4 = 128 * 8;
    extern __shared__ __attribute__((aligned(16))) unsigned char smem[];
    int count = d_count[0];
    if (count > max_count) count = max_count;
    const int b0 = blockIdx.x * GT_BS;
    if (b0 >= count) return;
    const int tid = threadIdx.x, lane = tid & 63;
    const int wave = __builtin_amdgcn_readfirstlane(tid >> 6);
    const int h = lane >> 5, sl = lane & 31;
    uint4* aring = (uint4*)smem + (size_t)wave * (GW_DA * AF * 64);
    uint4* ldsB = (uint4*)smem + (size_t)8 * GW_DA * AF * 64;
    const int nchunks = ksteps >> 1;
    const uint4* asrc = wp + (size_t)(wave * AF) * 64 + lane;
    const uint4* bsrc[2];
#pragma unroll
    for (int e = 0; e < 2; ++e) {
        const int s = 16 * wave + 8 * e + (lane >> 3);
        bsrc[e] = act + (size_t)(b0 + s) * act_row_u4 + (size_t)((lane & 7) ^ ((s >> 1) & 7));
    }
    auto issueA = [&](int kt, int slot) {
        kt = kt < ksteps ? kt : ksteps - 1;
#pragma unroll
        for (int i = 0; i < AF; ++i) dma16(asrc + (size_t)kt * (MT * 2 * 64) + i * 64, aring + (slot * AF + i) * 64);
    };
    auto issueA1 = [&](int kt, int slot, int i) {
        kt = kt < ksteps ? kt : ksteps - 1;
        dma16(asrc + (size_t)kt * (MT * 2 * 64) + i * 64, aring + (slot * AF + i) * 64);
    };
    auto issueB = [&](int ch, int buf) {
        ch = ch < nchunks ? ch : nchunks - 1;
#pragma unroll
        for (int e = 0; e < 2; ++e) dma16(bsrc[e] + ch * 8, ldsB + buf * B_U4 + (2 * wave + e) * 64);
    };
    f32x16 acc[MTW][4];
#pragma unroll
    for (int i = 0; i < MTW; ++i)
#pragma unroll
        for (int c = 0; c < 4; ++c)
#pragma unroll
// ... 163 lines not shown
}

static inline void split_h(float x, _Float16& hi, _Float16& lo) {
    hi = (_Float16)x;
    lo = (_Float16)(x - (float)hi);
}

template <typename GetW, typename KIdx>
static void pack_A(std::vector<_Float16>& out, int ksteps, int MT, GetW getw, KIdx kidx) {
    out.assign((size_t)ksteps * MT * 2 * 64 * 8, (_Float16)0.0f);
    for (int ks = 0; ks < ksteps; ++ks)
        for (int mt = 0; mt < MT; ++mt)
            for (int l = 0; l < 64; ++l)
                for (int j = 0; j < 8; ++j) {
                    const int r = l & 31, h = l >> 5;
                    const float w = getw(kidx(ks, h, j), 32 * mt + r);
                    _Float16 hi, lo;
                    split_h(w, hi, lo);
                    const size_t base = (((size_t)ks * MT + mt) * 2) * 512 + (size_t)l * 8 + j;
                    out[base] = hi;
                    out[base + 512] = lo;
                }
}

static uint8_t to_e2m3(float x) {
    const uint8_t sign = x < 0.0f ? 0x20 : 0x00;
    const float a = fabsf(x);
    if (!(a == a)) return sign;
    if (a >= 7.5f) return sign | 0x1f;
    int best = 0;
    float bd = 1e30f;
    for (int c = 0; c < 32; ++c) {
        const int ex = c >> 3, m = c & 7;
        const float v = ex == 0 ? m * 0.125f : (1.0f + m * 0.125f) * (float)(1 << (ex - 1));
        const float d = fabsf(v - a);
        if (d < bd || (d == bd && !(c & 1))) { bd = d; best = c; }
    }
    return sign | (uint8_t)best;
}
static int mx6_scale_byte(float amax) {
    if (!(amax > 0.0f)) return 1;
    int e;
    frexpf(amax * MX6_AMAX_ADJ, &e);
    int E = 127 + (e - 1) - 2;
    return E < 1 ? 1 : (E > 254 ? 254 : E);
}

static int heads_mt(int hw) { return ((hw + 1 + 31) / 32 + 3) / 4 * 4; }

const float* net_logits(const Net& net, int* row_stride) {
    if (net.mode == OMOK_NET_F32) { *row_stride = net.hw; return net.sh; }
    *row_stride = heads_mt(net.hw) * 32;
    return net.s0;
}

size_t net_alloc(Net& net) {
    const size_t hw = net.hw, rp = net.rowp;
    const size_t mb = ((size_t)net.max_b + GT_BS - 1) / GT_BS * GT_BS;
    size_t bytes = 0;
    auto A = [&](void** p, size_t n) {
        if (hipMalloc(p, n ? n : 16) != hipSuccess) return false;
        hipMemset(*p, 0, n ? n : 16);
        bytes += n;
        return true;
    };
    bool ok = true;
    for (int i = 0; i < NET_TENSORS && ok; ++i) ok = A((void**)&net.w[i], sizeof(float) * (size_t)net.wsize[i]);
    ok = ok && A((void**)&net.p, sizeof(float) * mb * rp);
    ok = ok && A((void**)&net.v, sizeof(float) * mb);
    ok = ok && A((void**)&net.vpre, sizeof(float) * mb);
    ok = ok && A((void**)&net.in_f32, sizeof(float) * mb * 3 * hw);
    net.cfg_mode = net.mode;
    if (net.mode == OMOK_NET_F32) {
        net.chunk = (int)std::min<size_t>(mb, 1024);
        const size_t c = net.chunk;
        ok = ok && A((void**)&net.sx, sizeof(float) * c * hw * NC);
        ok = ok && A((void**)&net.sh, sizeof(float) * c * hw * NM);
        ok = ok && A((void**)&net.sd, sizeof(float) * c * hw * NM);
        ok = ok && A((void**)&net.sg, sizeof(float) * c * hw * NM);
        ok = ok && A((void**)&net.s0, sizeof(float) * c * NF);
        ok = ok && A((void**)&net.s1, sizeof(float) * c * NF);
    } else {
        const size_t ks0 = hw * 8;
        const size_t row_pad = 80;
        net.row_u4_fmt[FC0_FP6] = (size_t)((hw + 31) / 32) * 2 * OP_BLK_U4 + row_pad;
        net.row_u4_fmt[FC0_F16] = (size_t)((hw + 31) / 32) * 2 * OPX_BLK_U4 + row_pad;
        net.row_u4 = net.row_u4_fmt[net.fc0_fmt];
        const size_t row_u4 = net.row_u4_fmt[FC0_F16];
        ok = ok && A(&net.wt_trunk, TR_WBYTES + TR_CONV_FRAGS * 1024);
        ok = ok && A((void**)&net.wt_first, sizeof(float) * (TR_SIDE_FLOATS + 2 * NF + heads_mt(net.hw) * 32));
        ok = ok && A(&net.wt_fc0, (ks0 + 4) * (size_t)MXS_FR * 1024);
        ok = ok && A(&net.wt_fc0x, (2 * ks0 + 8) * (size_t)X3_FR * 1024);
        ok = ok && A(&net.wt_fc1, (size_t)32 * 16 * 2 * 1024);
        ok = ok && A(&net.wt_heads, (size_t)32 * heads_mt(net.hw) * 2 * 1024);
        ok = ok && A(&net.a_fc0, mb * row_u4 * 16 + 2 * OPX_BLK_U4 * 16);
        ok = ok && A(&net.h0, mb * 32 * 64 * 2);
        ok = ok && A((void**)&net.s0, sizeof(float) * mb * heads_mt(net.hw) * 32);
        {
            ok = ok && A((void**)&net.d_groups, sizeof(uint2) * (mb / SIB_MIN + 1));
            ok = ok && A((void**)&net.d_singles, sizeof(int32_t) * mb);
            ok = ok && A((void**)&net.d_gcnt, sizeof(int32_t) * SIB_CNT_INTS);
            ok = ok && A((void**)&net.d_work, sizeof(unsigned long long) * NET_WORK_COUNT);
            if (ok) hipMemset(net.d_work, 0, sizeof(unsigned long long) * NET_WORK_COUNT);
            ok = ok && A((void**)&net.d_sib_rows, sizeof(uint4) * mb);
            net.base_slots = (size_t)SIB_WAYS * net.games + mb / SIB_MIN + 1;
            ok = ok && A((void**)&net.sib_h, net.base_slots * std::max<size_t>(sizeof(float) * 3 * (size_t)sib_hb_floats(net.n), sib2_slot_u4(net.n) * 16));
// ... 230 lines not shown
        const int MT = heads_mt(hw);
        pack_A(pk, 32, MT, [&](int k, int m) { return m < hw ? pw[(size_t)k * hw + m] : (m == hw ? vw[k] : 0.0f); },
               [](int ks, int h, int j) { return kperm(ks >> 1, ks & 1, h, j); });
        if (hipMemcpyAsync(net.wt_heads, pk.data(), pk.size() * 2, hipMemcpyHostToDevice, st) != hipSuccess) return -1;
        hipStreamSynchronize(st);
    }
    if (hipMemcpyAsync(net.wt_trunk, trunk.data(), trunk.size() * 2, hipMemcpyHostToDevice, st) != hipSuccess) return -1;
    if (hipMemcpyAsync(net.wt_first, side.data(), side.size() * 4, hipMemcpyHostToDevice, st) != hipSuccess) return -1;
    hipStreamSynchronize(st);
    return 0;
}

template <int N, bool FROM_F32, bool BASE = false, bool DELTA = false, bool F16LO = false>
static void launch_trunk(Net& net, const Store& S, int max_count, hipStream_t st, const int32_t* row_list = nullptr, const int32_t* d_nrows = nullptr,
                         const int32_t* d_out_base = nullptr, const int32_t* d_nrows2 = nullptr, bool v2 = false) {
    using TG = TrunkGeo<N>;
    static bool attr_done[64] = {};
    auto kern = k_trunk<N, FROM_F32, BASE, DELTA, F16LO>;
    if (!attr_done[net.device & 63]) {
        hipFuncSetAttribute((const void*)kern, hipFuncAttributeMaxDynamicSharedMemorySize, TG::LDS_BYTES);
        attr_done[net.device & 63] = true;
    }
    const int wgs = (max_count + TG::SPW - 1) / TG::SPW;
    const int grid = wgs < 256 ? wgs : 256;
    kern<<<grid, TG::WG_THREADS, TG::LDS_BYTES, st>>>(S.req_ref, S.req_aux, S.board, S.hdr, S.d_count, S.stride_nodes, net.in_f32, (const uint4*)net.wt_trunk, net.wt_first,
                                                       (uint4*)net.a_fc0, net.row_u4, max_count, row_list, d_nrows,
                                                       (BASE && DELTA) ? (const uint2*)net.d_comp : (const uint2*)net.d_groups, net.sib_h, d_out_base, (uint4*)net.a_base,
                                                       d_nrows2, v2 ? (uint4*)net.sib_h : nullptr);
}

template <int N, bool FROM_F32, bool BASE = false, bool DELTA = false>
static void launch_trunk_fmt(Net& net, const Store& S, int max_count, hipStream_t st, const int32_t* row_list = nullptr, const int32_t* d_nrows = nullptr,
                             const int32_t* d_out_base = nullptr, const int32_t* d_nrows2 = nullptr, bool v2 = false) {
    if (net.fc0_fmt == FC0_F16) launch_trunk<N, FROM_F32, BASE, DELTA, true>(net, S, max_count, st, row_list, d_nrows, d_out_base, d_nrows2, v2);
    else launch_trunk<N, FROM_F32, BASE, DELTA, false>(net, S, max_count, st, row_list, d_nrows, d_out_base, d_nrows2, v2);
}

template <int MT, int EPI, int TAG, int NST = 3>
static void launch_gemm(const void* wp, const void* act, int ksteps, size_t act_row_u4, int k_full, int last_cnt, int lo_off,
                        const float* bias, void* out_split, size_t out_row_u4, float* out_logits, const Store& S, int max_count,
                        hipStream_t st, int device, int nsplit = 1) {
    constexpr int LDS = (MT * 2 + 8) * 1024 * NST;
    static bool attr_done[64] = {};
    auto kern = k_gemm_t<MT, EPI, TAG, NST>;
    if (!attr_done[device & 63]) {
        hipFuncSetAttribute((const void*)kern, hipFuncAttributeMaxDynamicSharedMemorySize, LDS);
        attr_done[device & 63] = true;
    }
    const dim3 grid((max_count + GT_BS - 1) / GT_BS, nsplit);
    kern<<<grid, 512, LDS, st>>>((const uint4*)wp, (const uint4*)act, ksteps, act_row_u4, k_full, last_cnt, lo_off, bias, (uint4*)out_split,
                                  out_row_u4, out_logits, S.d_count, max_count);
}

template <int MTH>
static void launch_tail_fused(const void* wp_fc1, const void* act, const float* bias_fc1, const void* wp_heads, const float* bias_heads, float* out_logits, const Store& S,
                              int max_count, hipStream_t st, int device) {
    constexpr int LDS = 160 * 1024;
    static bool attr_done[64] = {};
    auto kern = k_tail_fused<MTH>;
    if (!attr_done[device & 63]) {
        hipFuncSetAttribute((const void*)kern, hipFuncAttributeMaxDynamicSharedMemorySize, LDS);
        attr_done[device & 63] = true;
    }
    kern<<<dim3((max_count + GT_BS - 1) / GT_BS), 512, LDS, st>>>((const uint4*)wp_fc1, (const uint4*)act, bias_fc1, (const uint4*)wp_heads, bias_heads, out_logits, S.d_count,
                                                                 max_count);
}

template <int MT, int EPI>
static void launch_gemm_w(const void* wp, const void* act, int ksteps, size_t act_row_u4, const float* bias, void* out_split, size_t out_row_u4, float* out_logits,
                          const Store& S, int max_count, hipStream_t st, int device) {
    constexpr int LDS = gemm_w_lds(MT);
    static_assert(LDS <= 160 * 1024, "k_gemm_w LDS");
    static bool attr_done[64] = {};
    auto kern = k_gemm_w<MT, EPI>;
    if (!attr_done[device & 63]) {
        hipFuncSetAttribute((const void*)kern, hipFuncAttributeMaxDynamicSharedMemorySize, LDS);
        attr_done[device & 63] = true;
    }
    kern<<<dim3((max_count + GT_BS - 1) / GT_BS), 512, LDS, st>>>((const uint4*)wp, (const uint4*)act, ksteps, act_row_u4, bias, (uint4*)out_split, out_row_u4, out_logits,
                                                                 S.d_count, max_count);
}

constexpr int SIB_MAX_WWAYS = 14;
constexpr int SIB_MAX_FWAYS = 64;
__global__ void k_zero_ints(int32_t* __restrict__ p, int n) {
    for (int i = threadIdx.x; i < n; i += blockDim.x) p[i] = 0;
}
typedef void (*sib_kernel_t)(const uint64_t*, const uint4*, const float*, uint4*, size_t, const uint4*, const int32_t*, const float*, const uint32_t*, const int32_t*,
                             uint4*, uint2*, unsigned long long*);
static sib_kernel_t sib_kernel(bool delta, bool x16, int n) {
    if (n == 9) return delta ? (x16 ? k_sib_children<true, true, 9> : k_sib_children<true, false, 9>)
                             : (x16 ? k_sib_children<false, true, 9> : k_sib_children<false, false, 9>);
    return delta ? (x16 ? k_sib_children<true, true, 15> : k_sib_children<true, false, 15>)
                 : (x16 ? k_sib_children<false, true, 15> : k_sib_children<false, false, 15>);
}
typedef void (*sib2_kernel_t)(const uint64_t*, const uint4*, const float*, uint4*, size_t, const uint4*, const int32_t*, const uint4*, const uint32_t*, const int32_t*,
                              uint4*, uint2*, unsigned long long*);
static sib2_kernel_t sib2_kernel(bool x16, int n, bool mixed = false) {
    if (mixed) return n == 9 ? k_sib_children2<true, 9, false, false> : k_sib_children2<true, 15, false, false>;
    if (n == 9) return x16 ? k_sib_children2<true, 9> : k_sib_children2<false, 9>;
    return x16 ? k_sib_children2<true, 15> : k_sib_children2<false, 15>;
}
static void launch_trunk_siblings(Net& net, const Store& S, int side, int max_count, hipStream_t st, bool delta) {
    constexpr int LDS = TR_WBYTES + 4 * SIB_CGRID_BYTES + TR_SIDE_FLOATS * 4;
    static_assert(LDS + 32 <= 160 * 1024, "k_sib_children LDS (+ the static pair-barrier flags)");
    static bool attr_done[64] = {};
    if (!attr_done[net.device & 63]) {
        for (int d = 0; d < 2; ++d)
            for (int x = 0; x < 2; ++x)
                for (int n : {9, 15}) hipFuncSetAttribute((const void*)sib_kernel(d != 0, x != 0, n), hipFuncAttributeMaxDynamicSharedMemorySize, LDS);
        for (int x = 0; x < 3; ++x)
            for (int n : {9, 15}) hipFuncSetAttribute((const void*)sib2_kernel(x != 0, n, x == 2), hipFuncAttributeMaxDynamicSharedMemorySize, V2_LDS);
        attr_done[net.device & 63] = true;
    }
    const bool x16 = net.fc0_fmt == FC0_F16;
    if (!net.gcnt_zeroed) k_zero_ints<<<1, 128, 0, st>>>(net.d_gcnt, SIB_CNT_INTS);
    const int do_fill = net.fill_in_group ? 1 : 0;
// ... 119 lines not shown
    const int stiles = wtiles_max < n_cu + 8 ? wtiles_max : n_cu + 8;
    launch_fc0<EPI_PARTIAL, true>(net, dfmt, n_cu + 8, st, net.d_rows, 0, drow_u4, bias_fc0, nullptr, net.part_w_rows, net.part_w, cnt, max_count, net.d_tile_info, net.d_slot_desc);
    k_win_finish<<<(unsigned)(((size_t)stiles * GT_BS * 64 + 255) / 256), 256, 0, st>>>(net.part_w, net.part_w_rows, cnt, net.d_tile_info, (const uint2*)net.d_slot_desc, net.facc,
                                                                                         bias_fc0, h0, 128);
}

static int sib_env() {
    static const int use_sib = getenv("OMOK_TRUNK_SIB") ? atoi(getenv("OMOK_TRUNK_SIB")) : 2;
    return use_sib;
}
static int sib_delta_min_rows(const Net& net) {
    static const int delta_min_env = getenv("OMOK_SIB_DELTA_MIN") ? atoi(getenv("OMOK_SIB_DELTA_MIN")) : 0;
    if (delta_min_env > 0) return delta_min_env;
    if (net.n != 15) return 1024;
    return net.diff_fp6 ? 2048 : 3072;
}
static bool sibling_path(const Net& net, bool from_f32, int sib_side) { return !from_f32 && sib_side >= 0 && sib_env() && net.siblings && net.d_groups; }
bool net_round_takes_sibling_path(const Net& net, int max_count) {
    if (net.mode == OMOK_NET_F32 || max_count <= 0) return false;
    return sibling_path(net, false, 0);
}
static void recover_handed_over_fill(Net& net, const Store& S, hipStream_t st, const char* where) {
    if (!net.fill_in_group) return;
    static bool said = false;
    if (!said) {
        said = true;
        fprintf(stderr, "omok_mi355x: internal inconsistency (recovered): the round's request-list fill was handed to the sibling path, but the forward (%s) does not take it; "
                        "the list is written here instead\n", where);
    }
    launch_fill(S, net.fill_side, net.fill_k, st);
    net.fill_in_group = net.gcnt_zeroed = false;
}
static int fc0_dense_nsplit(int rows, int nsup, int n_cu, size_t part_rows) {
    const int tiles128 = (rows + GT_BS - 1) / GT_BS;
    int nsplit = 1;
    double best = 1e30;
    constexpr int dmax = 64;
    for (int d = 1; d <= dmax; ++d) {
        const int per = (nsup + d - 1) / d;
        if ((d - 1) * per >= nsup) continue;
        if (d > 1 && (size_t)d * (size_t)(tiles128 * GT_BS) > part_rows) continue;
        const double waves = (double)(((size_t)tiles128 * d + n_cu - 1) / n_cu);
        const double cost = waves * (per + 4) * (d > 1 ? 1.04 : 1.0);
        if (cost < best - 1e-9) { best = cost; nsplit = d; }
    }
    return nsplit;
}
static int tail_tsplit(int rows, int n_cu, size_t part_rows) {
    const int tiles_t = (rows + GT_BS - 1) / GT_BS;
    int tsplit = 1;
    while (tsplit < 8 && tiles_t * tsplit * 2 <= n_cu && (size_t)(tsplit * 2) * (size_t)(tiles_t * GT_BS) <= part_rows) tsplit *= 2;
    return tsplit;
}
static void forward_f16x3(Net& net, const Store& S, int max_count, bool from_f32, hipStream_t st, Prof* prof, int sib_side = -1, bool skip_softmax = false) {
    const int hw = net.hw;
    const int use_sib = sib_env();
    const bool sib = sibling_path(net, from_f32, sib_side);
    if (!sib) recover_handed_over_fill(net, S, st, "forward_f16x3 on plain rows");
    const bool delta = sib && use_sib >= 2 && max_count >= sib_delta_min_rows(net);
    if (prof) prof->begin(PC_TRUNK, st);
    if (sib) launch_trunk_siblings(net, S, sib_side, max_count, st, delta);
    else if (net.n == 9) { if (from_f32) launch_trunk_fmt<9, true>(net, S, max_count, st); else launch_trunk_fmt<9, false>(net, S, max_count, st); }
    else {
        if (from_f32) launch_trunk_fmt<15, true>(net, S, max_count, st);
        else launch_trunk_fmt<15, false>(net, S, max_count, st);
    }
    if (prof) { prof->end(st); prof->begin(PC_FC0, st); }
    const float* bias_fc0 = net.wt_first + TR_SIDE_FLOATS;
    const float* bias_fc1 = bias_fc0 + NF;
    const float* bias_heads = bias_fc1 + NF;
    uint4* h0 = (uint4*)net.h0;
    const size_t mb = ((size_t)net.max_b + GT_BS - 1) / GT_BS * GT_BS;
    uint4* h1 = h0 + mb * 128;
    net.plan_path = sib ? (delta ? 2 : 1) : 0;
    net.plan_rows = max_count;
    net.plan_nsplit = 0;
    if (delta) launch_fc0_delta(net, max_count, bias_fc0, h0, st);
    else {
        const int nsup = hw * 2, tiles128 = (max_count + GT_BS - 1) / GT_BS;
        const int nsplit = net.plan_nsplit = fc0_dense_nsplit(max_count, nsup, net.n_cu, net.part_rows);
        if (nsplit == 1) launch_fc0<EPI_SPLIT, false>(net, net.fc0_fmt, tiles128, st, net.a_fc0, nsup, net.row_u4, bias_fc0, h0, 128, nullptr, S.d_count, max_count);
        else {
            const size_t cap_rows = (size_t)tiles128 * GT_BS;
            launch_fc0<EPI_PARTIAL, false>(net, net.fc0_fmt, (tiles128 * nsplit + 7) / 8 * 8, st, net.a_fc0, (nsup + nsplit - 1) / nsplit, net.row_u4, bias_fc0, nullptr, cap_rows,
                                           net.part, S.d_count, max_count);
            k_splitk_finish<<<(unsigned)(((size_t)max_count * 64 + 255) / 256), 256, 0, st>>>(net.part, nsplit, cap_rows, bias_fc0, h0, 128, S.d_count, max_count);
        }
    }
    if (prof) { prof->end(st); prof->begin(PC_TAIL, st); }
    const int MT = heads_mt(hw);
    const int tiles_t = (max_count + GT_BS - 1) / GT_BS;
    const int tsplit = net.plan_tsplit = tail_tsplit(max_count, net.n_cu, net.part_rows);
    const size_t cap_t = (size_t)tiles_t * GT_BS;
    const size_t fin_threads = (size_t)max_count * 64;
    if (tsplit == 1) {
        const char* gw_env = getenv("OMOK_GEMM_W");
        const bool gw = gw_env && gw_env[0] == '1';
        if (!gw) {
            if (MT == 8) launch_tail_fused<8>(net.wt_fc1, h0, bias_fc1, net.wt_heads, bias_heads, net.s0, S, max_count, st, net.device);
            else launch_tail_fused<4>(net.wt_fc1, h0, bias_fc1, net.wt_heads, bias_heads, net.s0, S, max_count, st, net.device);
        } else {
            launch_gemm_w<16, EPI_SPLIT>(net.wt_fc1, h0, 32, 128, bias_fc1, h1, 128, nullptr, S, max_count, st, net.device);
            if (MT == 8) launch_gemm_w<8, EPI_LOGITS>(net.wt_heads, h1, 32, 128, bias_heads, nullptr, 0, net.s0, S, max_count, st, net.device);
            else launch_gemm<4, EPI_LOGITS, 2>(net.wt_heads, h1, 32, 128, 32, 1, 2, bias_heads, nullptr, 0, net.s0, S, max_count, st, net.device);
        }
    } else {
        launch_gemm<16, EPI_PARTIAL, 1>(net.wt_fc1, h0, 32 / tsplit, 128, 32, 1, 2, bias_fc1, nullptr, cap_t, net.part, S, max_count, st, net.device, tsplit);
        k_splitk_finish<<<(unsigned)((fin_threads + 255) / 256), 256, 0, st>>>(net.part, tsplit, cap_t, bias_fc1, h1, 128, S.d_count, max_count);
        if (MT == 8) launch_gemm<8, EPI_PARTIAL, 2>(net.wt_heads, h1, 32 / tsplit, 128, 32, 1, 2, bias_heads, nullptr, cap_t, net.part, S, max_count, st, net.device, tsplit);
        else launch_gemm<4, EPI_PARTIAL, 2>(net.wt_heads, h1, 32 / tsplit, 128, 32, 1, 2, bias_heads, nullptr, cap_t, net.part, S, max_count, st, net.device, tsplit);
        const unsigned lg = (unsigned)(((size_t)max_count * (MT * 8) + 255) / 256);
        k_splitk_logits<<<lg < 2048 ? lg : 2048, 256, 0, st>>>(net.part, tsplit, cap_t, MT * 32, bias_heads, net.s0, S.d_count, max_count);
    }
    const int sg = max_count < 32768 ? max_count : 32768;
    if (!skip_softmax) k_softmax<<<sg, 64, 0, st>>>(net.s0, MT * 32, hw, net.rowp, net.p, net.v, net.vpre, S.d_count, max_count);
    if (prof) prof->end(st);
}

__device__ inline uint32_t probe_mix(uint32_t x) { x ^= x >> 16; x *= 0x7feb352dU; x ^= x >> 15; x *= 0x846ca68bU; x ^= x >> 16; return x; }
__global__ void k_probe_inputs(float* __restrict__ in, int hw, int rows, int row0) {
    const int i = blockIdx.x * blockDim.x + threadIdx.x;
    if (i >= rows * hw) return;
    const int r = i / hw, a = i % hw, gr = row0 + r;
    const uint32_t hr = probe_mix(0x9E3779B9u * (uint32_t)(gr + 1));
    const uint32_t kind = (uint32_t)gr % 5u;
    const uint32_t dens = kind < 2 ? (hr >> 8) % 40u : kind < 4 ? (hr >> 8) % 600u : (hr >> 8) % 1024u;
    const uint32_t hc = probe_mix(hr ^ (0x85EBCA6Bu * (uint32_t)(a + 1)));
    const bool occ = (hc & 1023u) < dens, black = (hc >> 10) & 1u;
    const int turn = (int)(hr & 1u);
    const bool mine = black == (turn == 0);
    float* o = in + (size_t)r * 3 * hw;
    o[2 * a] = occ && mine ? 1.0f : 0.0f;
    o[2 * a + 1] = occ && !mine ? 1.0f : 0.0f;
    o[2 * hw + a] = turn == 0 ? 1.0f : 0.0f;
}

__global__ __launch_bounds__(64) void k_probe_store(Store S, int n, int pk) {
    const int t = blockIdx.x, lane = threadIdx.x, hw = n * n, nw = (hw + 63) / 64;
    const uint32_t hr = probe_mix(0x9E3779B9u * (uint32_t)(t + 7919));
    const uint32_t kind = (uint32_t)t % 5u;
    const uint32_t dens = kind < 2 ? (hr >> 8) % 40u : (hr >> 8) % 500u;
    const int turn = (int)(hr & 1u);
    uint64_t bw[4] = {0, 0, 0, 0}, ww[4] = {0, 0, 0, 0};
    int stones = 0;
    for (int j = 0; j < nw; ++j) {
        const int a = j * 64 + lane;
        const uint32_t hc = probe_mix(hr ^ (0x85EBCA6Bu * (uint32_t)(a + 1)));
        const bool occ = a < hw && (hc & 1023u) < dens, black = (hc >> 10) & 1u;
        bw[j] = __ballot(occ && black);
        ww[j] = __ballot(occ && !black);
        stones += __popcll(bw[j] | ww[j]);
    }
    if (hw - stones <= pk) {
        for (int j = 0; j < 4; ++j) bw[j] = ww[j] = 0ULL;
        stones = 0;
    }
    const size_t tn = (size_t)t * (size_t)S.stride_nodes;
    const int legal = hw - stones;
    const int start = (int)((hr >> 3) % (uint32_t)hw);
    int found = 0;
    for (int k0 = 0; k0 < hw && found < pk; k0 += 64) {
        const int k = k0 + lane, c = (start + 7 * k) % hw;
        const bool empty = k < hw && !(((bw[c >> 6] | ww[c >> 6]) >> (c & 63)) & 1ULL);
        const unsigned long long m = __ballot(empty);
        const int idx = found + __popcll(m & ((1ULL << lane) - 1ULL));
        if (empty && idx < pk) {
            NodeHdr h;
            h.parent = 0; h.table = NONE16; h.legal = (uint16_t)(legal - 1); h.nch = 0; h.action = (uint8_t)c; h.status = ST_IN_PROGRESS;
            h.turn = (uint8_t)(1 - turn); h.has_policy = 0; h.pad = 0;
// ... 135 lines not shown
                            probe_acc(rounds[k].dp, rp_[k][row * rp + a], hp[2][(size_t)r * rp + a]);
                            probe_acc(rounds[k].dl, rl_[k][row * lrow + a], hl[(size_t)r * hw + a]);
                        }
                        probe_acc(rounds[k].dv, rv_[k][row], hv[2][r]);
                        probe_acc(rounds[k].dl, rl_[k][row * lrow + hw], hvp[2][r]);
                    }
                checked += b;
            }
            round_rows = rows;
        }
        for (int i = 0; i < 8; ++i) if (d[i]) hipFree(d[i]);
    }
    for (int i = 0; i < 6; ++i) if (tmp[i]) hipFree(tmp[i]);
    if (!ok) { net_set_fc0_format(net, fmt_before); return -1; }
    auto inside = [](const ProbeErr& e) { return e.dp <= NET_PROBE_LIMIT && e.dv <= NET_PROBE_LIMIT && e.dl <= NET_PROBE_LOGIT_LIMIT; };
    const bool have_rounds = round_rows > 0 && checked > 0;
    const bool fp6_ok = inside(plain[0]) && (!have_rounds || inside(rounds[0]));
    const bool mixed_ok = have_rounds && inside(rounds[1]);
    const int chosen = fp6_ok ? FC0_FP6 : mixed_ok ? FC0_MIXED : FC0_F16;
    net_set_fc0_format(net, chosen);
    auto contract = [](const ProbeErr& e) { return e.dp <= NET_PROBE_CONTRACT && e.dv <= NET_PROBE_CONTRACT && e.dl <= NET_PROBE_CONTRACT; };
    const ProbeErr& cp = plain[chosen == FC0_FP6 ? 0 : 1];
    const ProbeErr& cr = rounds[chosen == FC0_FP6 ? 0 : chosen == FC0_MIXED ? 1 : 2];
    net.probe_outside = (inside(cp) && (!have_rounds || inside(cr))) ? 0 : (contract(cp) && (!have_rounds || contract(cr))) ? 1 : 2;
    if (net.probe_outside) {
        static bool said[3] = {};
        if (!said[net.probe_outside]) {
            said[net.probe_outside] = true;
            fprintf(stderr, "omok_mi355x: net_commit: the %s operand format measures |dp| %.2e |dv| %.2e |dlogit| %.2e on plain rows%s against the fp32 kernels (max |logit| %.0f): %s\n",
                    chosen == FC0_FP6 ? "fp6" : chosen == FC0_MIXED ? "mixed" : "f16", cp.dp, cp.dv, cp.dl, have_rounds ? " (+ a sibling round)" : "", lmax,
                    net.probe_outside == 1 ? "outside the probe's margin (3e-4 / 5e-4), inside the 1e-3 contract -- committed (OMOK_STAT_PROBE_OUTSIDE = 1)"
                                           : "OUTSIDE the 1e-3 contract with the most precise split-operand format -- this net is evaluated with the fp32 kernels (slow; OMOK_STAT_PROBE_OUTSIDE = 2)");
        }
    }
    net.probe[0] = (float)R;
    net.probe[1] = plain[0].dp; net.probe[2] = plain[0].dv;
    net.probe[3] = plain[1].dp; net.probe[4] = plain[1].dv;
    net.probe[5] = lmax;
    net.probe[6] = 1.0f;
    net.probe[7] = plain[0].dl; net.probe[8] = plain[1].dl;
    net.probe[9] = (float)checked;
    for (int k = 0; k < 3; ++k) { net.probe[10 + 3 * k] = rounds[k].dp; net.probe[11 + 3 * k] = rounds[k].dv; net.probe[12 + 3 * k] = rounds[k].dl; }
    static const bool verbose = getenv("OMOK_PROBE_LOG") && atoi(getenv("OMOK_PROBE_LOG"));
    if (verbose)
        fprintf(stderr, "[net probe] N=%d plain rows %d: fp6 |dp| %.2e |dv| %.2e |dlogit| %.2e, f16 %.2e %.2e %.2e (max |logit| %.1f); sibling round of %d rows (%d checked): "
                        "fp6 %.2e %.2e %.2e, mixed %.2e %.2e %.2e, f16 %.2e %.2e %.2e -> %s\n", net.n, R, plain[0].dp, plain[0].dv, plain[0].dl, plain[1].dp, plain[1].dv, plain[1].dl,
                lmax, round_rows, checked, rounds[0].dp, rounds[0].dv, rounds[0].dl, rounds[1].dp, rounds[1].dv, rounds[1].dl, rounds[2].dp, rounds[2].dv, rounds[2].dl,
                chosen == FC0_FP6 ? "fp6" : chosen == FC0_MIXED ? "mixed" : "f16");
    return 0;
}

bool net_logits_cover_batch(const Net& net, int max_count) { return net.mode != OMOK_NET_F32 && max_count <= net.max_b; }

void net_forward_requests(Net& net, const Store& S, int max_count, hipStream_t st, Prof* prof, int sibling_side, bool skip_softmax) {
    if (max_count <= 0) return;
    if (max_count > net.max_b) max_count = net.max_b;
    if (net.mode == OMOK_NET_F32) {
        recover_handed_over_fill(net, S, st, "fp32 kernels");
        launch_encode_requests(net.n, S, net.in_f32, max_count, st);
        forward_f32(net, S, max_count, st, prof);
        net.plan_path = 3; net.plan_rows = max_count; net.plan_nsplit = net.plan_tsplit = 0;
    } else {
        forward_f16x3(net, S, max_count, false, st, prof, sibling_side, skip_softmax);
    }
}

void net_forward_inputs(Net& net, const Store& S, int count, hipStream_t st, Prof* prof) {
    if (count <= 0) return;
    if (net.mode == OMOK_NET_F32) {
        forward_f32(net, S, count, st, prof);
        net.plan_path = 3; net.plan_rows = count; net.plan_nsplit = net.plan_tsplit = 0;
    } else forward_f16x3(net, S, count, true, st, prof);
}

}
```

### omok-ai_amd/csrc/tree_kernels.hip

```cpp
#include "common.h"
#include <type_traits>

namespace omok {

#define LANE ((int)(threadIdx.x & 63))

struct U4 { uint32_t x, y, z, w; };

__device__ inline U4 philox(uint64_t seed, uint32_t c0, uint32_t c1, uint32_t c2, uint32_t c3) {
    uint32_t k0 = (uint32_t)seed, k1 = (uint32_t)(seed >> 32);
#pragma unroll
    for (int r = 0; r < 10; ++r) {
        const uint32_t h0 = __umulhi(0xD2511F53u, c0), l0 = 0xD2511F53u * c0;
        const uint32_t h1 = __umulhi(0xCD9E8D57u, c2), l1 = 0xCD9E8D57u * c2;
        const uint32_t n0 = h1 ^ c1 ^ k0, n2 = h0 ^ c3 ^ k1;
        c0 = n0; c1 = l1; c2 = n2; c3 = l0;
        k0 += 0x9E3779B9u;
        k1 += 0xBB67AE85u;
    }
    return U4{c0, c1, c2, c3};
}

__device__ inline double det_log(double x) {
    const unsigned long long b = (unsigned long long)__double_as_longlong(x);
    int e = (int)((b >> 52) & 0x7ff) - 1023;
    double m = __longlong_as_double((long long)((b & 0x000fffffffffffffULL) | 0x3ff0000000000000ULL));
    if (m > 1.4142135623730951) { m = m * 0.5; e = e + 1; }
    const double s = (m - 1.0) / (m + 1.0);
    const double s2 = s * s;
    double poly = 1.0 / 23.0;
    poly = poly * s2 + 1.0 / 21.0;
    poly = poly * s2 + 1.0 / 19.0;
    poly = poly * s2 + 1.0 / 17.0;
    poly = poly * s2 + 1.0 / 15.0;
    poly = poly * s2 + 1.0 / 13.0;
    poly = poly * s2 + 1.0 / 11.0;
    poly = poly * s2 + 1.0 / 9.0;
    poly = poly * s2 + 1.0 / 7.0;
    poly = poly * s2 + 1.0 / 5.0;
    poly = poly * s2 + 1.0 / 3.0;
    poly = poly * s2 + 1.0;
    const double lm = 2.0 * s * poly;
    return (double)e * 0.6931471805599453 + lm;
}

__device__ inline double pow2i(int k) { return __longlong_as_double((long long)(1023 + k) << 52); }

__device__ inline double det_exp(double x) {
    if (x > 709.0) return __longlong_as_double(0x7ff0000000000000LL);
    if (x < -745.0) return 0.0;
    const double t = x * 1.4426950408889634 + 0.5;
    long long ki = (long long)t;
    if ((double)ki > t) ki = ki - 1;
// ... 1125 lines not shown
            run += cnt[i];
        }
    }
    if (tid == 0) {
        S.d_count[0] = (int32_t)total;
        if (evals) evals[0] += total;
    }
}

__global__ __launch_bounds__(256) void k_fill(Store S, int side, int K) {
    const int i = blockIdx.x * 256 + threadIdx.x;
    const int g = i / K, r = i % K;
    if (g >= S.games || !S.gs[g].alive) return;
    const int t = side * S.games + g;
    const TreeState ts = S.ts[t];
    if ((uint32_t)r >= ts.n_req) return;
    S.req_ref[ts.req_base + r] = ((uint32_t)t << 16) | S.req_node[(size_t)t * KMAX + r];
    S.req_aux[ts.req_base + r] = 0xFFFFFFFFu;
}

template <int N>
__global__ __launch_bounds__(64) void k_scatter_policy(Store S, const float* __restrict__ P, int max_count) {
    using G = Geo<N>;
    constexpr int ROWP = G::ROWP, NW = G::NW;
    int count = S.d_count[0];
    if (count > max_count) count = max_count;
    const int lane = LANE;
    for (int d = blockIdx.x; d < count; d += gridDim.x) {
        const uint32_t ref = S.req_ref[d];
        const size_t tn = (size_t)(ref >> 16) * (size_t)S.stride_nodes + (size_t)(ref & 0xFFFFu);
        uint64_t occ[NW];
#pragma unroll
        for (int i = 0; i < NW; ++i) occ[i] = S.board[tn * (2 * NW) + i] | S.board[tn * (2 * NW) + NW + i];
        float row[G::IT];
#pragma unroll
        for (int j = 0; j < G::IT; ++j) {
            const int a = j * 64 + lane;
            const bool empty = a < G::HW && !((occ[j] >> lane) & 1ULL);
            row[j] = empty ? P[(size_t)d * ROWP + a] : 0.0f;
        }
        const float sum = seq_sum_regs<N>(row);
        const bool renorm = F32_EPS <= sum;
        const float inv = renorm ? __fdiv_rn(1.0f, sum) : 1.0f;
#pragma unroll
        for (int j = 0; j < G::IT; ++j) S.policy[tn * ROWP + j * 64 + lane] = renorm ? row[j] * inv : row[j];
        if (lane == 0) S.hdr[tn].has_policy = 1;
    }
}

#ifndef SSP_BATCH_N
#define SSP_BATCH_N 4
#endif
constexpr int SSP_BATCH = SSP_BATCH_N;
template <int N>
__global__ __launch_bounds__(64) void k_softmax_scatter_policy(Store S, const float* __restrict__ logits, int lrow, float* __restrict__ V,
                                                               float* __restrict__ Vpre, int max_count) {
    using G = Geo<N>;
    constexpr int ROWP = G::ROWP, NW = G::NW, hw = G::HW;
    static_assert((hw & 1) == 1, "odd row stride: conflict-free column reads");
    __shared__ float srow[SSP_BATCH * hw];
    __shared__ float sinv[SSP_BATCH];
    int count = S.d_count[0];
    if (count > max_count) count = max_count;
    const int lane = LANE;
    const int nb = (count + SSP_BATCH - 1) / SSP_BATCH;
    for (int b = blockIdx.x; b < nb; b += gridDim.x) {
        const int d0 = b * SSP_BATCH;
        const int nreq = count - d0 < SSP_BATCH ? count - d0 : SSP_BATCH;
        const uint32_t my_ref = lane < nreq ? S.req_ref[d0 + lane] : 0u;
        float lv[SSP_BATCH][G::IT];
#pragma unroll
        for (int i = 0; i < SSP_BATCH; ++i) {
            const float* l = logits + (size_t)(d0 + (i < nreq ? i : 0)) * lrow;
#pragma unroll
            for (int jj = 0; jj < G::IT; ++jj) lv[i][jj] = lane + 64 * jj < hw ? l[lane + 64 * jj] : -INFINITY;
        }
        const float my_vpre = lane < nreq ? logits[(size_t)(d0 + lane) * lrow + hw] : 0.0f;
        size_t tn[SSP_BATCH];
        uint64_t occ[SSP_BATCH][NW];
#pragma unroll
        for (int i = 0; i < SSP_BATCH; ++i) {
            const uint32_t ref = (uint32_t)__builtin_amdgcn_readlane((int)my_ref, i);
            tn[i] = (size_t)(ref >> 16) * (size_t)S.stride_nodes + (size_t)(ref & 0xFFFFu);
#pragma unroll
            for (int w = 0; w < NW; ++w) occ[i][w] = i < nreq ? (S.board[tn[i] * (2 * NW) + w] | S.board[tn[i] * (2 * NW) + NW + w]) : 0ULL;
        }
        if (lane < nreq) { V[d0 + lane] = tanhf(my_vpre); Vpre[d0 + lane] = my_vpre; }
#pragma unroll
        for (int i = 0; i < SSP_BATCH; ++i) {
            if (i < nreq) {
                float mx = -INFINITY;
#pragma unroll
                for (int jj = 0; jj < G::IT; ++jj) mx = fmaxf(mx, lv[i][jj]);
                for (int o = 32; o > 0; o >>= 1) mx = fmaxf(mx, __shfl_xor(mx, o, 64));
                float sum = 0.0f, row[G::IT];
#pragma unroll
                for (int jj = 0; jj < G::IT; ++jj) {
                    const int a = lane + 64 * jj;
                    row[jj] = 0.0f;
                    if (a < hw) { row[jj] = expf(lv[i][jj] - mx); sum += row[jj]; }
                }
                for (int o = 32; o > 0; o >>= 1) sum += __shfl_xor(sum, o, 64);
#pragma unroll
                for (int jj = 0; jj < G::IT; ++jj) {
                    const int a = jj * 64 + lane;
                    const float p = a < hw ? row[jj] / sum : 0.0f;
                    const bool empty = a < hw && !((occ[i][jj] >> lane) & 1ULL);
                    if (a < hw) srow[i * hw + a] = empty ? p : 0.0f;
                }
            }
        }
        __syncthreads();
        if (lane < nreq) {
            float acc = 0.0f;
#pragma unroll 15
            for (int a = 0; a < hw; ++a) acc += srow[lane * hw + a];
            const bool renorm = F32_EPS <= acc;
            sinv[lane] = renorm ? __fdiv_rn(1.0f, acc) : 0.0f;
        }
        __syncthreads();
#pragma unroll
        for (int i = 0; i < SSP_BATCH; ++i) {
            if (i < nreq) {
                const float inv = sinv[i];
                const bool renorm = inv != 0.0f;
#pragma unroll
                for (int jj = 0; jj < G::IT; ++jj) {
                    const int a = jj * 64 + lane;
                    const float r = a < hw ? srow[i * hw + a] : 0.0f;
                    S.policy[tn[i] * ROWP + a] = renorm ? r * inv : r;
                }
                if (lane == 0) S.hdr[tn[i]].has_policy = 1;
            }
        }
        __syncthreads();
    }
}

template <int N>
__device__ inline void scatter_tree(const Store& S, const Tree<N>& T, const TreeState& ts, Regs& R, const float* __restrict__ V) {
    using G = Geo<N>;
    constexpr int ROWP = G::ROWP;
    const int lane = LANE, nreq = (int)ts.n_req;
    int x = 0, par = -1 - lane, act = 0;
    float val = 0.0f;
    if (lane < nreq) {
        x = (int)T.req[lane];
        const NodeHdr hx = T.hdr[x];
        par = (int)hx.parent;
        act = (int)hx.action;
        val = V[(size_t)ts.req_base + lane];
    }
    const int prev_par = __shfl_up(par, 1, 64);
    unsigned long long rem = __ballot(lane < nreq && (lane == 0 || par != prev_par));
    while (rem) {
        const int s0 = __ffsll((long long)rem) - 1;
        rem &= rem - 1ULL;
        const int s1 = rem ? __ffsll((long long)rem) - 1 : nreq;
        const int leaf = __shfl(par, s0, 64);
        int depth = 0;
        size_t my_slot = 0;
        uint32_t my_n = 0;
        float my_w = 0.0f;
        bool fits = true;
        {
            int y = leaf;
            while (y != 0) {
                const NodeHdr h = T.hdr[y];
                const size_t slot = (size_t)T.hdr[h.parent].table * ROWP + h.action;
                const uint32_t n = T.cn[slot];
                const float w = T.cw[slot];
                if (lane == depth) { my_slot = slot; my_n = n; my_w = w; }
                y = h.parent;
                depth += 1;
                if (depth >= 64) { fits = y == 0; break; }
            }
        }
        if (fits) {
            const size_t tab_leaf = (size_t)T.hdr[leaf].table * ROWP;
            if (lane >= s0 && lane < s1) {
                const size_t slot = tab_leaf + act;
                const uint32_t n = T.cn[slot] + 1u;
                const float w = T.cw[slot] + (-val);
                T.cn[slot] = n;
                T.cw[slot] = w;
            }
            float root_w = R.root_w;
// ... 1169 lines not shown
                   (k_reset_from<15, true><<<2 * S.games, 64, 0, st>>>(S, boards, p, p2, split)));
    else
        DISPATCH_N(n, (k_reset_from<9, false><<<2 * S.games, 64, 0, st>>>(S, boards, p, nullptr, 0)),
                   (k_reset_from<15, false><<<2 * S.games, 64, 0, st>>>(S, boards, p, nullptr, 0)));
}
void launch_random_positions(int n, uint64_t key, int64_t first_game, int stones, int batch, uint8_t* boards, uint8_t* ok, hipStream_t st) {
    DISPATCH_N(n, (k_random_positions<9><<<batch, 64, 0, st>>>(key, first_game, stones, boards, ok)),
               (k_random_positions<15><<<batch, 64, 0, st>>>(key, first_game, stones, boards, ok)));
}
void launch_position_check(int n, const uint8_t* boards, int batch, int32_t* verdict, int32_t* stones, hipStream_t st) {
    DISPATCH_N(n, (k_position_check<9><<<batch, 64, 0, st>>>(boards, verdict, stones)), (k_position_check<15><<<batch, 64, 0, st>>>(boards, verdict, stones)));
}
void launch_log_move(int n, const Store& S, int side, int start_ply, const GameLog& L, hipStream_t st) {
    const int blocks = (S.games + 255) / 256;
    DISPATCH_N(n, (k_log_move<9><<<blocks, 256, 0, st>>>(S, side, start_ply, L)), (k_log_move<15><<<blocks, 256, 0, st>>>(S, side, start_ply, L)));
}
void launch_replay(int n, const uint8_t* start, const int32_t* verdict, const uint16_t* moves, const int32_t* lengths, int batch, int stride, int upto,
                   uint8_t* boards_out, int32_t* status_out, int32_t* played_out, hipStream_t st) {
    DISPATCH_N(n, (k_replay<9><<<batch, 64, 0, st>>>(start, verdict, moves, lengths, stride, upto, boards_out, status_out, played_out)),
               (k_replay<15><<<batch, 64, 0, st>>>(start, verdict, moves, lengths, stride, upto, boards_out, status_out, played_out)));
}
void launch_root_stats(const Store& S, int side, uint32_t* n_dev, float* w_dev, hipStream_t st) {
    k_root_stats<<<(S.games + 255) / 256, 256, 0, st>>>(S, side, n_dev, w_dev);
}
void launch_round(int n, const Store& S, const RoundArgs& a, hipStream_t st) {
    DISPATCH_N(n, (k_round<9><<<S.games, 64, 0, st>>>(S, a)), (k_round<15><<<S.games, 64, 0, st>>>(S, a)));
}
void launch_round_shared(int n, const Store& S, const RoundArgs& a, int rounds_total, int group, int waves, uint16_t* sh_req, uint32_t* sh_cnt,
                         hipStream_t st, uint8_t* rec_order, uint32_t* rec_pos) {
    DISPATCH_N(n, (k_round_shared<9><<<1, waves * 64, 0, st>>>(S, a, rounds_total, group, sh_req, sh_cnt, rec_order, rec_pos)),
               (k_round_shared<15><<<1, waves * 64, 0, st>>>(S, a, rounds_total, group, sh_req, sh_cnt, rec_order, rec_pos)));
    k_scan_shared<<<1, 64, 0, st>>>(S, a.side, waves, sh_req, sh_cnt);
}
void launch_scatter_shared(int n, const Store& S, int side, const float* p, const float* v, int max_count, int waves, const uint16_t* sh_req,
                           const uint32_t* sh_cnt, hipStream_t st, uint8_t* rec_order, uint32_t* rec_pos) {
    const int grid = max_count > 0 ? max_count : 1;
    DISPATCH_N(n, (k_scatter_policy<9><<<grid, 64, 0, st>>>(S, p, max_count)), (k_scatter_policy<15><<<grid, 64, 0, st>>>(S, p, max_count)));
    DISPATCH_N(n, (k_scatter_shared<9><<<1, waves * 64, 0, st>>>(S, side, v, sh_req, sh_cnt, rec_order, rec_pos)),
               (k_scatter_shared<15><<<1, waves * 64, 0, st>>>(S, side, v, sh_req, sh_cnt, rec_order, rec_pos)));
}
void launch_fill(const Store& S, int side, int K, hipStream_t st) { k_fill<<<(S.games * K + 255) / 256, 256, 0, st>>>(S, side, K); }
void launch_scan(int n, const Store& S, int side, int K, hipStream_t st, unsigned long long* evals, int32_t* zero_ptr, int zero_n, bool fill) {
    k_scan<<<1, 1024, 0, st>>>(S, side, evals, zero_ptr, zero_ptr ? zero_n : 0);
    if (fill) launch_fill(S, side, K, st);
}
void launch_scatter(int n, const Store& S, int side, const float* p, const float* v, int max_count, hipStream_t st, bool backups) {
    const int grid = max_count < 8192 ? (max_count > 0 ? max_count : 1) : 8192;
    DISPATCH_N(n, (k_scatter_policy<9><<<grid, 64, 0, st>>>(S, p, max_count)), (k_scatter_policy<15><<<grid, 64, 0, st>>>(S, p, max_count)));
    if (backups) launch_backups(n, S, side, v, st);
}
void launch_backups(int n, const Store& S, int side, const float* v, hipStream_t st) {
    DISPATCH_N(n, (k_scatter<9><<<S.games, 64, 0, st>>>(S, side, v)), (k_scatter<15><<<S.games, 64, 0, st>>>(S, side, v)));
}
void launch_softmax_scatter(int n, const Store& S, int side, const float* logits, int lrow, float* v, float* vpre, int max_count, hipStream_t st,
                            bool backups) {
    const int nb = (max_count + SSP_BATCH - 1) / SSP_BATCH;
    const int grid = nb < 8192 ? (nb > 0 ? nb : 1) : 8192;
    DISPATCH_N(n, (k_softmax_scatter_policy<9><<<grid, 64, 0, st>>>(S, logits, lrow, v, vpre, max_count)),
               (k_softmax_scatter_policy<15><<<grid, 64, 0, st>>>(S, logits, lrow, v, vpre, max_count)));
    if (backups) launch_backups(n, S, side, v, st);
}
void launch_sample(int n, const Store& S, int side, int ply, float temperature, int threshold, uint64_t seed,
                   int64_t game_offset, int32_t* actions, hipStream_t st) {
    DISPATCH_N(n, (k_sample<9><<<S.games, 64, 0, st>>>(S, side, ply, temperature, threshold, seed, game_offset, actions)),
               (k_sample<15><<<S.games, 64, 0, st>>>(S, side, ply, temperature, threshold, seed, game_offset, actions)));
}
void launch_mirror_scan(int n, const Store& S, int side, hipStream_t st) { k_mirror_scan<<<1, 1024, 0, st>>>(S, side); }
void launch_advance(int n, const Store& S, int side, const float* p, hipStream_t st) {
    const size_t lds = advance_lds_bytes(S.cap_nodes, S.cap_tables);
    DISPATCH_N(n, (k_advance<9><<<S.games, 64, lds, st>>>(S, side, p)), (k_advance<15><<<S.games, 64, lds, st>>>(S, side, p)));
}
void launch_encode_requests(int n, const Store& S, float* out, int max_b, hipStream_t st) {
    if (max_b <= 0) return;
    DISPATCH_N(n, (k_encode_requests<9><<<max_b, 256, 0, st>>>(S, out, max_b)), (k_encode_requests<15><<<max_b, 256, 0, st>>>(S, out, max_b)));
}
void launch_env_play(int n, const int32_t* moves, int batch, int len, int32_t* status, uint8_t* boards, uint8_t* turns,
                     uint16_t* legal, hipStream_t st) {
    DISPATCH_N(n, (k_env_play<9><<<batch, 64, 0, st>>>(moves, len, status, boards, turns, legal)),
               (k_env_play<15><<<batch, 64, 0, st>>>(moves, len, status, boards, turns, legal)));
}
void launch_encode_boards(int n, const uint8_t* boards, const uint8_t* turns, int batch, int mode, float* out, hipStream_t st) {
    DISPATCH_N(n, (k_encode_boards<9><<<batch, 256, 0, st>>>(boards, turns, mode, out)),
               (k_encode_boards<15><<<batch, 256, 0, st>>>(boards, turns, mode, out)));
}
void launch_replay_offsets(int n, const Store& S, int per_transition, long long* offsets, hipStream_t st) {
    DISPATCH_N(n, (k_replay_offsets<9><<<1, 64, 0, st>>>(S, per_transition, offsets)), (k_replay_offsets<15><<<1, 64, 0, st>>>(S, per_transition, offsets)));
}
void launch_set_actions(int n, const Store& S, int side, const int32_t* actions, uint32_t* flags, hipStream_t st) {
    const int grid = (S.games + 255) / 256;
    DISPATCH_N(n, (k_set_actions<9><<<grid, 256, 0, st>>>(S, side, actions, flags)), (k_set_actions<15><<<grid, 256, 0, st>>>(S, side, actions, flags)));
}
void launch_clear_actions(const Store& S, hipStream_t st) { k_clear_actions<<<(S.games + 255) / 256, 256, 0, st>>>(S); }
void launch_opponent_move(int n, const Store& S, int side, int kind, uint64_t seed, int64_t game_offset, int32_t* actions, hipStream_t st) {
    DISPATCH_N(n, (k_opponent_move<9><<<S.games, 64, 0, st>>>(S, side, kind, seed, game_offset, actions)),
               (k_opponent_move<15><<<S.games, 64, 0, st>>>(S, side, kind, seed, game_offset, actions)));
}
void launch_env_scripted(int n, const uint8_t* boards, int kind, int batch, int32_t* forced, hipStream_t st) {
    DISPATCH_N(n, (k_env_scripted<9><<<batch, 64, 0, st>>>(boards, kind, forced)), (k_env_scripted<15><<<batch, 64, 0, st>>>(boards, kind, forced)));
}
void launch_policy(int n, const Store& S, int side, float* pi, uint8_t* has, hipStream_t st) {
    DISPATCH_N(n, (k_policy<9><<<S.games, 64, 0, st>>>(S, side, pi, has)), (k_policy<15><<<S.games, 64, 0, st>>>(S, side, pi, has)));
}
void launch_env_place(int n, uint8_t* boards, uint8_t* turns, uint16_t* legal, const int32_t* actions, int batch, int32_t* status, hipStream_t st) {
    DISPATCH_N(n, (k_env_place<9><<<batch, 64, 0, st>>>(boards, turns, legal, actions, status)),
               (k_env_place<15><<<batch, 64, 0, st>>>(boards, turns, legal, actions, status)));
}
int set_advance_lds_attribute(int n, size_t bytes) {
    const void* f = n == 9 ? (const void*)k_advance<9> : (const void*)k_advance<15>;
    return hipFuncSetAttribute(f, hipFuncAttributeMaxDynamicSharedMemorySize, (int)bytes) == hipSuccess ? 0 : -1;
}
void launch_replay_augment(int n, const Store& S, const long long* offsets, int game_first, int game_count, long long base_sub,
                           uint8_t* dst, long long cap, hipStream_t st) {
// ... 33 lines not shown
```

Before: 586.6 games/s.

## Fuse masked policy softmax and scatter into the fused tail kernel epilogue

The fused tail kernel (fc1 plus heads) can now stage its logits tile in LDS and perform the masked softmax, renormalisation, value tanh and policy store into the tree directly, instead of writing logits to global memory for a separate softmax-scatter kernel. Occupancy words for each request are prefetched mid-GEMM so the epilogue has them ready. The standalone softmax-scatter kernel also learns to sum split-K partial logits plus bias, which removes a separate reduction pass when the tail is split. This saves a kernel launch and a logits round trip per round, at the cost of a heavier epilogue and extra LDS and register pressure in the tail kernel.

```diff
diff --git a/bindings/omok_mi355x.rs b/bindings/omok_mi355x.rs
--- a/bindings/omok_mi355x.rs
+++ b/bindings/omok_mi355x.rs
@@ -180,6 +180,8 @@
         pub fn omok_debug_set_base_cache(e: *mut OmokEngine, enabled: i32) -> c_int;
         pub fn omok_debug_set_children_kernel(e: *mut OmokEngine, which: i32) -> c_int;
         pub fn omok_debug_set_window_rects(e: *mut OmokEngine, enabled: i32) -> c_int;
+        pub fn omok_debug_set_tail_scatter(e: *mut OmokEngine, enabled: i32) -> c_int;
+        pub fn omok_debug_tail_scatter_rounds(e: *const OmokEngine) -> i64;
         pub fn omok_debug_last_plan(e: *mut OmokEngine, out: *mut i32, cap: i32) -> c_int;
         pub fn omok_get_stats(e: *mut OmokEngine, stats: *mut f64) -> c_int;
         pub fn omok_reset_stats(e: *mut OmokEngine) -> c_int;
diff --git a/include/omok_mi355x.h b/include/omok_mi355x.h
--- a/include/omok_mi355x.h
+++ b/include/omok_mi355x.h
@@ -156,6 +156,8 @@
 int omok_debug_set_base_cache(omok_engine* e, int32_t enabled);
 int omok_debug_set_children_kernel(omok_engine* e, int32_t which);
 int omok_debug_set_window_rects(omok_engine* e, int32_t enabled);
+int omok_debug_set_tail_scatter(omok_engine* e, int32_t enabled);
+int64_t omok_debug_tail_scatter_rounds(const omok_engine* e);
 #define OMOK_PLAN_INTS 16
 int omok_debug_last_plan(omok_engine* e, int32_t* out, int32_t cap);
 
diff --git a/omok-ai_amd/api.py b/omok-ai_amd/api.py
--- a/omok-ai_amd/api.py
+++ b/omok-ai_amd/api.py
@@ -233,6 +233,12 @@
 
     def set_window_rects(self, on=True):
         self._chk(B.lib().omok_debug_set_window_rects(self.h, int(bool(on))))
+
+    def set_tail_scatter(self, on=True):
+        self._chk(B.lib().omok_debug_set_tail_scatter(self.h, int(bool(on))))
+
+    def tail_scatter_rounds(self):
+        return int(self._chk(B.lib().omok_debug_tail_scatter_rounds(self.h)))
 
     def set_children_kernel(self, which=2):
         self._chk(B.lib().omok_debug_set_children_kernel(self.h, int(which)))
diff --git a/omok-ai_amd/binding.py b/omok-ai_amd/binding.py
--- a/omok-ai_amd/binding.py
+++ b/omok-ai_amd/binding.py
@@ -35,7 +35,7 @@
     "omok_round_eval", "omok_round_outputs", "omok_round_logits", "omok_round_inject", "omok_round_scatter", "omok_mirror_generate",
     "omok_mirror_inputs", "omok_mirror_eval", "omok_mirror_outputs", "omok_mirror_inject", "omok_mirror_apply",
     "omok_alive_count", "omok_current_ply", "omok_game_info", "omok_tree_dump", "omok_tree_root", "omok_replay_game",
-    "omok_operand_row_bytes", "omok_debug_operand_rows", "omok_debug_set_base_cache", "omok_debug_set_children_kernel", "omok_debug_set_window_rects", "omok_debug_last_plan",
+    "omok_operand_row_bytes", "omok_debug_operand_rows", "omok_debug_set_base_cache", "omok_debug_set_children_kernel", "omok_debug_set_window_rects", "omok_debug_set_tail_scatter", "omok_debug_tail_scatter_rounds", "omok_debug_last_plan",
     "omok_replay_pack_dev", "omok_replay_record_bytes", "omok_replay_augment_dev", "omok_replay_augmented_game", "omok_get_stats", "omok_reset_stats", "omok_set_profiling",
     "omok_train_begin", "omok_train_end", "omok_train_step", "omok_train_losses", "omok_train_batch_indices", "omok_train_run",
     "omok_train_gradient_count", "omok_train_backward", "omok_train_apply",
@@ -102,6 +102,9 @@
     L.omok_debug_set_base_cache.argtypes = [H, C.c_int32]
     L.omok_debug_set_children_kernel.argtypes = [H, C.c_int32]
     L.omok_debug_set_window_rects.argtypes = [H, C.c_int32]
+    L.omok_debug_set_tail_scatter.argtypes = [H, C.c_int32]
+    L.omok_debug_tail_scatter_rounds.argtypes = [H]
+    L.omok_debug_tail_scatter_rounds.restype = C.c_int64
     L.omok_debug_last_plan.argtypes = [H, ip, C.c_int32]
     L.omok_set_episode.argtypes = [H, C.c_uint64]
     L.omok_env_place_stone.argtypes = [H, u8p, u8p, C.POINTER(C.c_uint16), ip, C.c_int32, ip]
diff --git a/omok-ai_amd/csrc/common.h b/omok-ai_amd/csrc/common.h
--- a/omok-ai_amd/csrc/common.h
+++ b/omok-ai_amd/csrc/common.h
@@ -124,7 +124,7 @@
 void launch_scatter(int n, const Store& S, int side, const float* p_dev, const float* v_dev, int max_count, hipStream_t st, bool backups = true);
 void launch_backups(int n, const Store& S, int side, const float* v_dev, hipStream_t st);
 void launch_softmax_scatter(int n, const Store& S, int side, const float* logits_dev, int lrow, float* v_dev, float* vpre_dev, int max_count,
-                            hipStream_t st, bool backups = true);
+                            hipStream_t st, bool backups = true, int nsplit = 0, size_t split_stride = 0, const float* bias_dev = nullptr);
 void launch_sample(int n, const Store& S, int side, int ply, float temperature, int threshold, uint64_t seed,
                    int64_t game_offset, int32_t* actions_dev, hipStream_t st);
 void launch_mirror_scan(int n, const Store& S, int side, hipStream_t st);
diff --git a/omok-ai_amd/csrc/engine.cpp b/omok-ai_amd/csrc/engine.cpp
--- a/omok-ai_amd/csrc/engine.cpp
+++ b/omok-ai_amd/csrc/engine.cpp
@@ -339,6 +339,7 @@
     HIPCHK(e, hipMemset(e->d_mevals, 0, 16));
     Net* n2 = new Net();
     configure_net(e, *n2, e->net.max_b);
+    n2->tail_scatter = e->net.tail_scatter;
     if (net_alloc(*n2) == 0) { delete n2; return fail(e, OMOK_ERR_HIP, "net 2 buffer allocation failed (hipMalloc)"); }
     e->net2 = n2;
     return 0;
@@ -499,14 +500,16 @@
     else { V.req_ref = e->d_mref; V.req_aux = e->d_maux; V.d_count = e->d_mcnt + 1; }
     return V;
 }
-static void match_forward(omok_engine* e, int b, int tree_side, int max_count, int sibling_side, bool skip_softmax) {
+static bool match_forward(omok_engine* e, int b, int tree_side, int max_count, int sibling_side, bool skip_softmax, bool scatter = false) {
     Net& X = net_at(e, tree_side ^ b);
     X.grp_lo = b ? e->split : 0;
     X.grp_hi = b ? e->cfg.games : e->split;
     X.grp_sub = b ? e->d_mcnt : nullptr;
-    net_forward_requests(X, block_view(e, b), max_count, e->st, &e->prof, sibling_side, skip_softmax);
+    const bool scattered = net_forward_requests(X, block_view(e, b), max_count, e->st, &e->prof, sibling_side, skip_softmax, scatter ? X.v : nullptr,
+                                                scatter ? X.vpre : nullptr);
     X.grp_hi = -1;
     X.grp_sub = nullptr;
+    return scattered;
 }
 static void match_split(omok_engine* e, int tree_side, int max_rows) {
     launch_match_split(e->S, tree_side, e->split, e->d_mref, e->d_maux, e->d_mcnt, e->d_mevals, max_rows, e->st);
@@ -1000,12 +1003,11 @@
         Net& X = net_at(e, side ^ b);
         const Store V = block_view(e, b);
         const bool fused = net_logits_cover_batch(X, alive * K);
-        match_forward(e, b, side, alive * K, side, fused);
+        if (match_forward(e, b, side, alive * K, side, fused, fused)) continue;
         e->prof.begin(PC_TREE_OTHER, e->st);
         if (fused) {
-            int lrow = 0;
-            const float* lg = net_logits(X, &lrow);
-            launch_softmax_scatter(e->n, V, side, lg, lrow, X.v, X.vpre, alive * K, e->st, false);
+            const NetLogitsRef lg = net_logits_ref(X);
+            launch_softmax_scatter(e->n, V, side, lg.rows, lg.row_stride, X.v, X.vpre, alive * K, e->st, false, lg.nsplit, lg.split_stride, lg.bias);
         } else launch_scatter(e->n, V, side, X.p, X.v, alive * K, e->st, false);
         e->prof.end(e->st);
     }
@@ -1041,12 +1043,13 @@
     e->prof.end(e->st);
     if (eval_and_scatter) {
         const bool fused = net_logits_cover_batch(e->net, alive * K);
-        net_forward_requests(e->net, e->S, alive * K, e->st, &e->prof, side, fused);
+        const bool scattered = net_forward_requests(e->net, e->S, alive * K, e->st, &e->prof, side, fused, fused ? e->net.v : nullptr, fused ? e->net.vpre : nullptr);
         e->prof.begin(PC_TREE_OTHER, e->st);
-        if (fused) {
-            int lrow = 0;
-            const float* lg = net_logits(e->net, &lrow);
-            launch_softmax_scatter(e->n, e->S, side, lg, lrow, e->net.v, e->net.vpre, alive * K, e->st, !defer_backups);
+        if (scattered) {
+            if (!defer_backups) launch_backups(e->n, e->S, side, e->net.v, e->st);
+        } else if (fused) {
+            const NetLogitsRef lg = net_logits_ref(e->net);
+            launch_softmax_scatter(e->n, e->S, side, lg.rows, lg.row_stride, e->net.v, e->net.vpre, alive * K, e->st, !defer_backups, lg.nsplit, lg.split_stride, lg.bias);
         } else launch_scatter(e->n, e->S, side, e->net.p, e->net.v, alive * K, e->st, !defer_backups);
         e->prof.end(e->st);
     }
@@ -2061,6 +2064,18 @@
     if (!e) return OMOK_ERR_INVALID;
     e->net.win_rects = enabled != 0;
     return OMOK_OK;
+}
+
+extern "C" int omok_debug_set_tail_scatter(omok_engine* e, int32_t enabled) {
+    if (!e) return OMOK_ERR_INVALID;
+    e->net.tail_scatter = enabled != 0;
+    if (e->net2) e->net2->tail_scatter = enabled != 0;
+    return OMOK_OK;
+}
+
+extern "C" int64_t omok_debug_tail_scatter_rounds(const omok_engine* e) {
+    if (!e) return OMOK_ERR_INVALID;
+    return (int64_t)(e->net.tail_scatter_rounds + (e->net2 ? e->net2->tail_scatter_rounds : 0));
 }
 
 extern "C" int omok_debug_set_children_kernel(omok_engine* e, int32_t which) {
diff --git a/omok-ai_amd/csrc/net.h b/omok-ai_amd/csrc/net.h
--- a/omok-ai_amd/csrc/net.h
+++ b/omok-ai_amd/csrc/net.h
@@ -66,6 +66,7 @@
     double children_launches[2] = {0.0, 0.0};
     bool sib_v2 = true;
     bool win_rects = true;
+    bool tail_scatter = true;
     bool base_cache = true;
     bool sib_cache_valid = false;
     float* part_w = nullptr;
@@ -82,6 +83,9 @@
     int grp_lo = 0, grp_hi = -1;
     const int32_t* grp_sub = nullptr;
     int plan_path = -1, plan_rows = 0, plan_nsplit = 0, plan_tsplit = 0;
+    int logits_nsplit = 0;
+    size_t logits_split_stride = 0;
+    long long tail_scatter_rounds = 0;
 };
 
 inline int64_t net_tensor_size(int n, int idx) {
@@ -126,12 +130,15 @@
 constexpr int NET_GCNT_P0 = 8 + 81 + 7 + 16;
 constexpr int NET_GCNT_INTS = NET_GCNT_P0 + 225;
 constexpr int NET_WORK_DIFF = 0, NET_WORK_COPY = 3, NET_WORK_DIFF_FULL = 6, NET_WORK_WIN_PIXELS = 7, NET_WORK_WIN_TILES = 8, NET_WORK_FULL_TILES = 9, NET_WORK_COUNT = 16;
-void net_forward_requests(Net& net, const Store& S, int max_count, hipStream_t st, struct Prof* prof, int sibling_side = -1, bool skip_softmax = false);
+bool net_forward_requests(Net& net, const Store& S, int max_count, hipStream_t st, struct Prof* prof, int sibling_side = -1, bool skip_softmax = false,
+                          float* scatter_v = nullptr, float* scatter_vpre = nullptr);
 void net_forward_inputs(Net& net, const Store& S, int count, hipStream_t st, struct Prof* prof);
 inline void net_invalidate_sibling_cache(Net& net) { net.sib_cache_valid = false; }
 int net_commit(Net& net, const Store& S, hipStream_t st);
 void net_set_fc0_format(Net& net, int fmt);
 const float* net_logits(const Net& net, int* row_stride);
+struct NetLogitsRef { const float* rows; int row_stride; int nsplit; size_t split_stride; const float* bias; };
+NetLogitsRef net_logits_ref(const Net& net);
 size_t net_alloc(Net& net);
 void net_free(Net& net);
 
diff --git a/omok-ai_amd/csrc/net_kernels.hip b/omok-ai_amd/csrc/net_kernels.hip
--- a/omok-ai_amd/csrc/net_kernels.hip
+++ b/omok-ai_amd/csrc/net_kernels.hip
@@ -1,4 +1,5 @@
 #include "net.h"
+#include "policy_scatter.h"
 
 #include <cmath>
 #include <cstdlib>
@@ -2595,10 +2596,11 @@
     }
 }
 
-template <int MTH>
+template <int MTH, int SN>
 __global__ __launch_bounds__(512) void k_tail_fused(const uint4* __restrict__ wp_fc1, const uint4* __restrict__ act, const float* __restrict__ bias_fc1,
                                                     const uint4* __restrict__ wp_heads, const float* __restrict__ bias_heads, float* __restrict__ out_logits,
-                                                    const int32_t* __restrict__ d_count, int max_count) {
+                                                    Store S, float* __restrict__ V, float* __restrict__ Vpre, int max_count) {
+    const int32_t* __restrict__ d_count = S.d_count;
     constexpr int MTW = MTH / 4;
     constexpr int WFR = MTH * 2;
     constexpr int LPW = WFR / 8;
@@ -2657,6 +2659,18 @@
         }
     }
 
+    constexpr int TS_N = SN > 0 ? SN : 15;
+    constexpr int TS_NW = Geo<TS_N>::NW;
+    int ts_nreq = 0;
+    uint32_t ts_ref = 0u;
+    uint64_t ts_occ = 0ULL;
+    if constexpr (SN > 0) {
+        static_assert(16 * TS_NW <= 64 && TS_N * TS_N + 1 <= MTH * 32, "one occupancy word per lane; policy and value columns inside the heads' tile");
+        ts_nreq = count - (b0 + 16 * wave);
+        ts_nreq = ts_nreq < 0 ? 0 : ts_nreq > 16 ? 16 : ts_nreq;
+        if (lane < ts_nreq) ts_ref = S.req_ref[b0 + 16 * wave + lane];
+    }
+
     f32x16 acc[MTW][2];
 #pragma unroll
     for (int i = 0; i < MTW; ++i)
@@ -2671,6 +2685,12 @@
             asm volatile("s_waitcnt lgkmcnt(0)" ::: "memory");
             __builtin_amdgcn_s_barrier();
             asm volatile("" ::: "memory");
+        }
+        if constexpr (SN > 0) {
+            if (p == 3) {
+                const uint32_t ref = (uint32_t)__shfl((int)ts_ref, lane / TS_NW, 64);
+                if (lane < ts_nreq * TS_NW) ts_occ = ssp_occ_word<TS_N>(S, ssp_node(S, ref), lane % TS_NW);
+            }
         }
         if (wm == p) {
 #pragma unroll
@@ -2719,20 +2739,76 @@
         }
     }
 
-#pragma unroll
-    for (int c = 0; c < 2; ++c) {
-        const int sample = b0 + 32 * (2 * ws + c) + (lane & 31);
-        if (sample >= count) continue;
-#pragma unroll
-        for (int i = 0; i < MTW; ++i) {
-            const int mt = wm * MTW + i;
-#pragma unroll
-            for (int g = 0; g < 4; ++g) {
-                const f32x4 bv = *(const f32x4*)(bias_heads + 32 * mt + 8 * g + 4 * h);
-                f32x4 o;
-#pragma unroll
-                for (int q = 0; q < 4; ++q) o[q] = acc[i][c][4 * g + q] + bv[q];
-                *(f32x4*)(out_logits + (size_t)sample * (MTH * 32) + 32 * mt + 8 * g + 4 * h) = o;
+    if constexpr (SN == 0) {
+#pragma unroll
+        for (int c = 0; c < 2; ++c) {
+            const int sample = b0 + 32 * (2 * ws + c) + (lane & 31);
+            if (sample >= count) continue;
+#pragma unroll
+            for (int i = 0; i < MTW; ++i) {
+                const int mt = wm * MTW + i;
+#pragma unroll
+                for (int g = 0; g < 4; ++g) {
+                    const f32x4 bv = *(const f32x4*)(bias_heads + 32 * mt + 8 * g + 4 * h);
+                    f32x4 o;
+#pragma unroll
+                    for (int q = 0; q < 4; ++q) o[q] = acc[i][c][4 * g + q] + bv[q];
+                    *(f32x4*)(out_logits + (size_t)sample * (MTH * 32) + 32 * mt + 8 * g + 4 * h) = o;
+                }
+            }
+        }
+    } else {
+        using G = Geo<TS_N>;
+        constexpr int hw = G::HW, TS_LSTR = MTH * 32 + 4;
+        static_assert(GT_BS * TS_LSTR * 4 <= 160 * 1024 && (TS_LSTR * 4) % 16 == 0, "the tile fits the LDS; rows 16-B aligned");
+        float* tile = (float*)smem;
+        asm volatile("s_waitcnt lgkmcnt(0)" ::: "memory");
+        __builtin_amdgcn_s_barrier();
+        asm volatile("" ::: "memory");
+#pragma unroll
+        for (int c = 0; c < 2; ++c) {
+            float* trow = tile + (32 * (2 * ws + c) + (lane & 31)) * TS_LSTR;
+#pragma unroll
+            for (int i = 0; i < MTW; ++i) {
+                const int mt = wm * MTW + i;
+#pragma unroll
+                for (int g = 0; g < 4; ++g) {
+                    const f32x4 bv = *(const f32x4*)(bias_heads + 32 * mt + 8 * g + 4 * h);
+                    f32x4 o;
+#pragma unroll
+                    for (int q = 0; q < 4; ++q) o[q] = acc[i][c][4 * g + q] + bv[q];
+                    *(f32x4*)(trow + 32 * mt + 8 * g + 4 * h) = o;
+                }
+            }
+        }
+        asm volatile("s_waitcnt lgkmcnt(0)" ::: "memory");
+        __builtin_amdgcn_s_barrier();
+        asm volatile("" ::: "memory");
+        if (ts_nreq > 0) {
+            const int d0 = b0 + 16 * wave;
+            float* rows = tile + 16 * wave * TS_LSTR;
+            if (lane < ts_nreq) ssp_store_value(V, Vpre, d0 + lane, rows[lane * TS_LSTR + hw]);
+            for (int i = 0; i < ts_nreq; ++i) {
+                float* row = rows + i * TS_LSTR;
+                float lv[G::IT], out[G::IT];
+                ssp_load_row<TS_N>(SspRow{row}, lane, lv);
+                uint64_t occ[TS_NW];
+#pragma unroll
+                for (int w = 0; w < TS_NW; ++w)
+                    occ[w] = (uint64_t)(uint32_t)__builtin_amdgcn_readlane((int)(uint32_t)ts_occ, i * TS_NW + w) |
+                             (uint64_t)(uint32_t)__builtin_amdgcn_readlane((int)(uint32_t)(ts_occ >> 32), i * TS_NW + w) << 32;
+                ssp_masked_softmax<TS_N>(lv, occ, lane, out);
+#pragma unroll
+                for (int jj = 0; jj < G::IT; ++jj)
+                    if (jj * 64 + lane < hw) row[jj * 64 + lane] = out[jj];
+            }
+            asm volatile("s_waitcnt lgkmcnt(0)" ::: "memory");
+            __builtin_amdgcn_wave_barrier();
+            float inv = 0.0f;
+            if (lane < ts_nreq) inv = ssp_row_inv<TS_N>(rows + lane * TS_LSTR);
+            for (int i = 0; i < ts_nreq; ++i) {
+                const size_t tn = ssp_node(S, (uint32_t)__builtin_amdgcn_readlane((int)ts_ref, i));
+                ssp_store_row<TS_N>(S, tn, rows + i * TS_LSTR, __int_as_float(__builtin_amdgcn_readlane(__float_as_int(inv), i)), lane);
             }
         }
     }
@@ -3002,6 +3078,18 @@
     if (net.mode == OMOK_NET_F32) { *row_stride = net.hw; return net.sh; }
     *row_stride = heads_mt(net.hw) * 32;
     return net.s0;
+}
+
+NetLogitsRef net_logits_ref(const Net& net) {
+    NetLogitsRef r{};
+    if (net.mode != OMOK_NET_F32 && net.logits_nsplit > 0) {
+        r.rows = net.part;
+        r.row_stride = heads_mt(net.hw) * 32;
+        r.nsplit = net.logits_nsplit;
+        r.split_stride = net.logits_split_stride;
+        r.bias = net.wt_first + TR_SIDE_FLOATS + 2 * NF;
+    } else r.rows = net_logits(net, &r.row_stride);
+    return r;
 }
 
 size_t net_alloc(Net& net) {
@@ -3338,17 +3426,17 @@
                                   out_row_u4, out_logits, S.d_count, max_count);
 }
 
-template <int MTH>
+template <int MTH, int SN>
 static void launch_tail_fused(const void* wp_fc1, const void* act, const float* bias_fc1, const void* wp_heads, const float* bias_heads, float* out_logits, const Store& S,
-                              int max_count, hipStream_t st, int device) {
+                              float* v, float* vpre, int max_count, hipStream_t st, int device) {
     constexpr int LDS = 160 * 1024;
     static bool attr_done[64] = {};
-    auto kern = k_tail_fused<MTH>;
+    auto kern = k_tail_fused<MTH, SN>;
     if (!attr_done[device & 63]) {
         hipFuncSetAttribute((const void*)kern, hipFuncAttributeMaxDynamicSharedMemorySize, LDS);
         attr_done[device & 63] = true;
     }
-    kern<<<dim3((max_count + GT_BS - 1) / GT_BS), 512, LDS, st>>>((const uint4*)wp_fc1, (const uint4*)act, bias_fc1, (const uint4*)wp_heads, bias_heads, out_logits, S.d_count,
+    kern<<<dim3((max_count + GT_BS - 1) / GT_BS), 512, LDS, st>>>((const uint4*)wp_fc1, (const uint4*)act, bias_fc1, (const uint4*)wp_heads, bias_heads, out_logits, S, v, vpre,
                                                                  max_count);
 }
 
@@ -3574,7 +3662,9 @@
     while (tsplit < 8 && tiles_t * tsplit * 2 <= n_cu && (size_t)(tsplit * 2) * (size_t)(tiles_t * GT_BS) <= part_rows) tsplit *= 2;
     return tsplit;
 }
-static void forward_f16x3(Net& net, const Store& S, int max_count, bool from_f32, hipStream_t st, Prof* prof, int sib_side = -1, bool skip_softmax = false) {
+static bool forward_f16x3(Net& net, const Store& S, int max_count, bool from_f32, hipStream_t st, Prof* prof, int sib_side = -1, bool skip_softmax = false,
+                          float* scatter_v = nullptr, float* scatter_vpre = nullptr) {
+    bool scattered = false;
     const int hw = net.hw;
     const int use_sib = sib_env();
     const bool sib = sibling_path(net, from_f32, sib_side);
@@ -3613,14 +3703,20 @@
     const int MT = heads_mt(hw);
     const int tiles_t = (max_count + GT_BS - 1) / GT_BS;
     const int tsplit = net.plan_tsplit = tail_tsplit(max_count, net.n_cu, net.part_rows);
+    net.logits_nsplit = 0;
     const size_t cap_t = (size_t)tiles_t * GT_BS;
     const size_t fin_threads = (size_t)max_count * 64;
     if (tsplit == 1) {
         const char* gw_env = getenv("OMOK_GEMM_W");
         const bool gw = gw_env && gw_env[0] == '1';
-        if (!gw) {
-            if (MT == 8) launch_tail_fused<8>(net.wt_fc1, h0, bias_fc1, net.wt_heads, bias_heads, net.s0, S, max_count, st, net.device);
-            else launch_tail_fused<4>(net.wt_fc1, h0, bias_fc1, net.wt_heads, bias_heads, net.s0, S, max_count, st, net.device);
+        scattered = !gw && skip_softmax && net.tail_scatter && scatter_v && scatter_vpre && (net.n == 15 || net.n == 9);
+        if (scattered) {
+            ++net.tail_scatter_rounds;
+            if (net.n == 15) launch_tail_fused<8, 15>(net.wt_fc1, h0, bias_fc1, net.wt_heads, bias_heads, net.s0, S, scatter_v, scatter_vpre, max_count, st, net.device);
+            else launch_tail_fused<4, 9>(net.wt_fc1, h0, bias_fc1, net.wt_heads, bias_heads, net.s0, S, scatter_v, scatter_vpre, max_count, st, net.device);
+        } else if (!gw) {
+            if (MT == 8) launch_tail_fused<8, 0>(net.wt_fc1, h0, bias_fc1, net.wt_heads, bias_heads, net.s0, S, nullptr, nullptr, max_count, st, net.device);
+            else launch_tail_fused<4, 0>(net.wt_fc1, h0, bias_fc1, net.wt_heads, bias_heads, net.s0, S, nullptr, nullptr, max_count, st, net.device);
         } else {
             launch_gemm_w<16, EPI_SPLIT>(net.wt_fc1, h0, 32, 128, bias_fc1, h1, 128, nullptr, S, max_count, st, net.device);
             if (MT == 8) launch_gemm_w<8, EPI_LOGITS>(net.wt_heads, h1, 32, 128, bias_heads, nullptr, 0, net.s0, S, max_count, st, net.device);
@@ -3631,12 +3727,18 @@
         k_splitk_finish<<<(unsigned)((fin_threads + 255) / 256), 256, 0, st>>>(net.part, tsplit, cap_t, bias_fc1, h1, 128, S.d_count, max_count);
         if (MT == 8) launch_gemm<8, EPI_PARTIAL, 2>(net.wt_heads, h1, 32 / tsplit, 128, 32, 1, 2, bias_heads, nullptr, cap_t, net.part, S, max_count, st, net.device, tsplit);
         else launch_gemm<4, EPI_PARTIAL, 2>(net.wt_heads, h1, 32 / tsplit, 128, 32, 1, 2, bias_heads, nullptr, cap_t, net.part, S, max_count, st, net.device, tsplit);
-        const unsigned lg = (unsigned)(((size_t)max_count * (MT * 8) + 255) / 256);
-        k_splitk_logits<<<lg < 2048 ? lg : 2048, 256, 0, st>>>(net.part, tsplit, cap_t, MT * 32, bias_heads, net.s0, S.d_count, max_count);
+        if (skip_softmax && net.tail_scatter && scatter_v && scatter_vpre && (tsplit == 2 || tsplit == 4 || tsplit == 8)) {
+            net.logits_nsplit = tsplit;
+            net.logits_split_stride = cap_t * (size_t)(MT * 32);
+        } else {
+            const unsigned lg = (unsigned)(((size_t)max_count * (MT * 8) + 255) / 256);
+            k_splitk_logits<<<lg < 2048 ? lg : 2048, 256, 0, st>>>(net.part, tsplit, cap_t, MT * 32, bias_heads, net.s0, S.d_count, max_count);
+        }
     }
     const int sg = max_count < 32768 ? max_count : 32768;
     if (!skip_softmax) k_softmax<<<sg, 64, 0, st>>>(net.s0, MT * 32, hw, net.rowp, net.p, net.v, net.vpre, S.d_count, max_count);
     if (prof) prof->end(st);
+    return scattered;
 }
 
 __device__ inline uint32_t probe_mix(uint32_t x) { x ^= x >> 16; x *= 0x7feb352dU; x ^= x >> 15; x *= 0x846ca68bU; x ^= x >> 16; return x; }
@@ -3878,8 +3980,9 @@
 
 bool net_logits_cover_batch(const Net& net, int max_count) { return net.mode != OMOK_NET_F32 && max_count <= net.max_b; }
 
-void net_forward_requests(Net& net, const Store& S, int max_count, hipStream_t st, Prof* prof, int sibling_side, bool skip_softmax) {
-    if (max_count <= 0) return;
+bool net_forward_requests(Net& net, const Store& S, int max_count, hipStream_t st, Prof* prof, int sibling_side, bool skip_softmax, float* scatter_v,
+                          float* scatter_vpre) {
+    if (max_count <= 0) return false;
     if (max_count > net.max_b) max_count = net.max_b;
     if (net.mode == OMOK_NET_F32) {
         recover_handed_over_fill(net, S, st, "fp32 kernels");
@@ -3887,8 +3990,9 @@
         forward_f32(net, S, max_count, st, prof);
         net.plan_path = 3; net.plan_rows = max_count; net.plan_nsplit = net.plan_tsplit = 0;
     } else {
-        forward_f16x3(net, S, max_count, false, st, prof, sibling_side, skip_softmax);
-    }
+        return forward_f16x3(net, S, max_count, false, st, prof, sibling_side, skip_softmax, scatter_v, scatter_vpre);
+    }
+    return false;
 }
 
 void net_forward_inputs(Net& net, const Store& S, int count, hipStream_t st, Prof* prof) {
diff --git a/omok-ai_amd/csrc/policy_scatter.h b/omok-ai_amd/csrc/policy_scatter.h
--- /dev/null
+++ b/omok-ai_amd/csrc/policy_scatter.h
@@ -0,0 +1,96 @@
+#pragma once
+#include "common.h"
+
+namespace omok {
+
+__device__ inline size_t ssp_node(const Store& S, uint32_t ref) { return (size_t)(ref >> 16) * (size_t)S.stride_nodes + (size_t)(ref & 0xFFFFu); }
+
+template <int N>
+__device__ inline uint64_t ssp_occ_word(const Store& S, size_t tn, int w) {
+    constexpr int NW = Geo<N>::NW;
+    return S.board[tn * (2 * NW) + w] | S.board[tn * (2 * NW) + NW + w];
+}
+
+struct SspRow {
+    const float* p;
+    __device__ float operator()(int a) const { return p[a]; }
+};
+
+template <int NS>
+struct SspPartialRow {
+    const float* p;
+    size_t split_stride;
+    const float* bias;
+    __device__ float operator()(int a) const {
+#pragma clang fp contract(off)
+        float x = p[a];
+#pragma unroll
+        for (int sp = 1; sp < NS; ++sp) x += p[(size_t)sp * split_stride + a];
+        x += bias[a];
+        return x;
+    }
+};
+
+template <int N, class Logit>
+__device__ inline void ssp_load_row(const Logit& logit, int lane, float (&lv)[Geo<N>::IT]) {
+#pragma unroll
+    for (int jj = 0; jj < Geo<N>::IT; ++jj) lv[jj] = lane + 64 * jj < Geo<N>::HW ? logit(lane + 64 * jj) : -INFINITY;
+}
+
+template <int N>
+__device__ inline void ssp_masked_softmax(const float (&lv)[Geo<N>::IT], const uint64_t (&occ)[Geo<N>::NW], int lane, float (&out)[Geo<N>::IT]) {
+#pragma clang fp contract(off)
+    using G = Geo<N>;
+    constexpr int hw = G::HW;
+    float mx = -INFINITY;
+#pragma unroll
+    for (int jj = 0; jj < G::IT; ++jj) mx = fmaxf(mx, lv[jj]);
+    for (int o = 32; o > 0; o >>= 1) mx = fmaxf(mx, __shfl_xor(mx, o, 64));
+    float sum = 0.0f, row[G::IT];
+#pragma unroll
+    for (int jj = 0; jj < G::IT; ++jj) {
+        const int a = lane + 64 * jj;
+        row[jj] = 0.0f;
+        if (a < hw) { row[jj] = expf(lv[jj] - mx); sum += row[jj]; }
+    }
+    for (int o = 32; o > 0; o >>= 1) sum += __shfl_xor(sum, o, 64);
+#pragma unroll
+    for (int jj = 0; jj < G::IT; ++jj) {
+        const int a = jj * 64 + lane;
+        const float p = a < hw ? row[jj] / sum : 0.0f;
+        const bool empty = a < hw && !((occ[jj] >> lane) & 1ULL);
+        out[jj] = empty ? p : 0.0f;
+    }
+}
+
+template <int N>
+__device__ inline float ssp_row_inv(const float* row) {
+#pragma clang fp contract(off)
+    float acc = 0.0f;
+#pragma unroll 15
+    for (int a = 0; a < Geo<N>::HW; ++a) acc += row[a];
+    const bool renorm = F32_EPS <= acc;
+    return renorm ? __fdiv_rn(1.0f, acc) : 0.0f;
+}
+
+template <int N>
+__device__ inline void ssp_store_row(const Store& S, size_t tn, const float* row, float inv, int lane) {
+#pragma clang fp contract(off)
+    using G = Geo<N>;
+    const bool renorm = inv != 0.0f;
+#pragma unroll
+    for (int jj = 0; jj < G::IT; ++jj) {
+        const int a = jj * 64 + lane;
+        const float r = a < G::HW ? row[a] : 0.0f;
+        S.policy[tn * G::ROWP + a] = renorm ? r * inv : r;
+    }
+    if (lane == 0) S.hdr[tn].has_policy = 1;
+}
+
+__device__ inline void ssp_store_value(float* __restrict__ V, float* __restrict__ Vpre, int d, float vpre) {
+#pragma clang fp contract(off)
+    V[d] = tanhf(vpre);
+    Vpre[d] = vpre;
+}
+
+}
diff --git a/omok-ai_amd/csrc/tree_kernels.hip b/omok-ai_amd/csrc/tree_kernels.hip
--- a/omok-ai_amd/csrc/tree_kernels.hip
+++ b/omok-ai_amd/csrc/tree_kernels.hip
@@ -1,4 +1,6 @@
 #include "common.h"
+#include "policy_scatter.h"
+#include <cstdio>
 #include <type_traits>
 
 namespace omok {
@@ -1230,11 +1232,11 @@
 #define SSP_BATCH_N 4
 #endif
 constexpr int SSP_BATCH = SSP_BATCH_N;
-template <int N>
+template <int N, int NS>
 __global__ __launch_bounds__(64) void k_softmax_scatter_policy(Store S, const float* __restrict__ logits, int lrow, float* __restrict__ V,
-                                                               float* __restrict__ Vpre, int max_count) {
-    using G = Geo<N>;
-    constexpr int ROWP = G::ROWP, NW = G::NW, hw = G::HW;
+                                                               float* __restrict__ Vpre, int max_count, size_t split_stride, const float* __restrict__ bias) {
+    using G = Geo<N>;
+    constexpr int NW = G::NW, hw = G::HW;
     static_assert((hw & 1) == 1, "odd row stride: conflict-free column reads");
     __shared__ float srow[SSP_BATCH * hw];
     __shared__ float sinv[SSP_BATCH];
@@ -1250,67 +1252,40 @@
 #pragma unroll
         for (int i = 0; i < SSP_BATCH; ++i) {
             const float* l = logits + (size_t)(d0 + (i < nreq ? i : 0)) * lrow;
-#pragma unroll
-            for (int jj = 0; jj < G::IT; ++jj) lv[i][jj] = lane + 64 * jj < hw ? l[lane + 64 * jj] : -INFINITY;
-        }
-        const float my_vpre = lane < nreq ? logits[(size_t)(d0 + lane) * lrow + hw] : 0.0f;
+            if constexpr (NS == 0) ssp_load_row<N>(SspRow{l}, lane, lv[i]);
+            else ssp_load_row<N>(SspPartialRow<NS>{l, split_stride, bias}, lane, lv[i]);
+        }
+        float my_vpre = 0.0f;
+        if (lane < nreq) {
+            const float* l = logits + (size_t)(d0 + lane) * lrow;
+            if constexpr (NS == 0) my_vpre = SspRow{l}(hw);
+            else my_vpre = SspPartialRow<NS>{l, split_stride, bias}(hw);
+        }
         size_t tn[SSP_BATCH];
         uint64_t occ[SSP_BATCH][NW];
 #pragma unroll
         for (int i = 0; i < SSP_BATCH; ++i) {
-            const uint32_t ref = (uint32_t)__builtin_amdgcn_readlane((int)my_ref, i);
-            tn[i] = (size_t)(ref >> 16) * (size_t)S.stride_nodes + (size_t)(ref & 0xFFFFu);
-#pragma unroll
-            for (int w = 0; w < NW; ++w) occ[i][w] = i < nreq ? (S.board[tn[i] * (2 * NW) + w] | S.board[tn[i] * (2 * NW) + NW + w]) : 0ULL;
-        }
-        if (lane < nreq) { V[d0 + lane] = tanhf(my_vpre); Vpre[d0 + lane] = my_vpre; }
+            tn[i] = ssp_node(S, (uint32_t)__builtin_amdgcn_readlane((int)my_ref, i));
+#pragma unroll
+            for (int w = 0; w < NW; ++w) occ[i][w] = i < nreq ? ssp_occ_word<N>(S, tn[i], w) : 0ULL;
+        }
+        if (lane < nreq) ssp_store_value(V, Vpre, d0 + lane, my_vpre);
 #pragma unroll
         for (int i = 0; i < SSP_BATCH; ++i) {
             if (i < nreq) {
-                float mx = -INFINITY;
-#pragma unroll
-                for (int jj = 0; jj < G::IT; ++jj) mx = fmaxf(mx, lv[i][jj]);
-                for (int o = 32; o > 0; o >>= 1) mx = fmaxf(mx, __shfl_xor(mx, o, 64));
-                float sum = 0.0f, row[G::IT];
-#pragma unroll
-                for (int jj = 0; jj < G::IT; ++jj) {
-                    const int a = lane + 64 * jj;
-                    row[jj] = 0.0f;
-                    if (a < hw) { row[jj] = expf(lv[i][jj] - mx); sum += row[jj]; }
-                }
-                for (int o = 32; o > 0; o >>= 1) sum += __shfl_xor(sum, o, 64);
-#pragma unroll
-                for (int jj = 0; jj < G::IT; ++jj) {
-                    const int a = jj * 64 + lane;
-                    const float p = a < hw ? row[jj] / sum : 0.0f;
-                    const bool empty = a < hw && !((occ[i][jj] >> lane) & 1ULL);
-                    if (a < hw) srow[i * hw + a] = empty ? p : 0.0f;
-                }
+                float out[G::IT];
+                ssp_masked_softmax<N>(lv[i], occ[i], lane, out);
+#pragma unroll
+                for (int jj = 0; jj < G::IT; ++jj)
+                    if (jj * 64 + lane < hw) srow[i * hw + jj * 64 + lane] = out[jj];
             }
         }
         __syncthreads();
-        if (lane < nreq) {
-            float acc = 0.0f;
-#pragma unroll 15
-            for (int a = 0; a < hw; ++a) acc += srow[lane * hw + a];
-            const bool renorm = F32_EPS <= acc;
-            sinv[lane] = renorm ? __fdiv_rn(1.0f, acc) : 0.0f;
-        }
+        if (lane < nreq) sinv[lane] = ssp_row_inv<N>(srow + lane * hw);
         __syncthreads();
 #pragma unroll
-        for (int i = 0; i < SSP_BATCH; ++i) {
-            if (i < nreq) {
-                const float inv = sinv[i];
-                const bool renorm = inv != 0.0f;
-#pragma unroll
-                for (int jj = 0; jj < G::IT; ++jj) {
-                    const int a = jj * 64 + lane;
-                    const float r = a < hw ? srow[i * hw + a] : 0.0f;
-                    S.policy[tn[i] * ROWP + a] = renorm ? r * inv : r;
-                }
-                if (lane == 0) S.hdr[tn[i]].has_policy = 1;
-            }
-        }
+        for (int i = 0; i < SSP_BATCH; ++i)
+            if (i < nreq) ssp_store_row<N>(S, tn[i], srow + i * hw, sinv[i], lane);
         __syncthreads();
     }
 }
@@ -2586,12 +2561,24 @@
 void launch_backups(int n, const Store& S, int side, const float* v, hipStream_t st) {
     DISPATCH_N(n, (k_scatter<9><<<S.games, 64, 0, st>>>(S, side, v)), (k_scatter<15><<<S.games, 64, 0, st>>>(S, side, v)));
 }
-void launch_softmax_scatter(int n, const Store& S, int side, const float* logits, int lrow, float* v, float* vpre, int max_count, hipStream_t st,
-                            bool backups) {
+template <int NS>
+static void launch_ssp(int n, const Store& S, const float* logits, int lrow, float* v, float* vpre, int max_count, hipStream_t st, size_t split_stride, const float* bias) {
     const int nb = (max_count + SSP_BATCH - 1) / SSP_BATCH;
     const int grid = nb < 8192 ? (nb > 0 ? nb : 1) : 8192;
-    DISPATCH_N(n, (k_softmax_scatter_policy<9><<<grid, 64, 0, st>>>(S, logits, lrow, v, vpre, max_count)),
-               (k_softmax_scatter_policy<15><<<grid, 64, 0, st>>>(S, logits, lrow, v, vpre, max_count)));
+    DISPATCH_N(n, (k_softmax_scatter_policy<9, NS><<<grid, 64, 0, st>>>(S, logits, lrow, v, vpre, max_count, split_stride, bias)),
+               (k_softmax_scatter_policy<15, NS><<<grid, 64, 0, st>>>(S, logits, lrow, v, vpre, max_count, split_stride, bias)));
+}
+void launch_softmax_scatter(int n, const Store& S, int side, const float* logits, int lrow, float* v, float* vpre, int max_count, hipStream_t st,
+                            bool backups, int nsplit, size_t split_stride, const float* bias) {
+    switch (nsplit) {
+        case 0: launch_ssp<0>(n, S, logits, lrow, v, vpre, max_count, st, 0, nullptr); break;
+        case 2: launch_ssp<2>(n, S, logits, lrow, v, vpre, max_count, st, split_stride, bias); break;
+        case 4: launch_ssp<4>(n, S, logits, lrow, v, vpre, max_count, st, split_stride, bias); break;
+        case 8: launch_ssp<8>(n, S, logits, lrow, v, vpre, max_count, st, split_stride, bias); break;
+        default:
+            fprintf(stderr, "omok_mi355x: internal inconsistency: launch_softmax_scatter got %d-way partials; the round's policies are NOT scattered\n", nsplit);
+            return;
+    }
     if (backups) launch_backups(n, S, side, v, st);
 }
 void launch_sample(int n, const Store& S, int side, int ply, float temperature, int threshold, uint64_t seed,
```

New measurement: 590.3 games/s (median of 6 runs). No clear change (+0.6%).
